# EricBAndrews/Fast-Needleman-Wunsch

Measured on AMD Instinct MI355X. Metric: GCUPS (DP cell updates/s) on NxN NW fill, bit-exact score, higher is better.
Workload: dtype int32; 1 GPU; nw_fill_262144x262144; n1=262144, n2=262144, table_bytes=274880004100, layout=row-major int32, pitch 262208, waves=auto, parallelism=single GPU, kernel=panels

## Files before the change

### fast-needleman-wunsch_amd/csrc/nw_capi.cpp

```cpp
#include <cstring>

#include "nw_host_int.h"

using namespace nwh;

extern "C" {

void nw_params_default(nw_params *p) {
    if (!p) return;
    std::memset(p, 0, sizeof(*p));
    p->match = 1;
    p->mismatch = 0;
    p->gap = -1;
    p->mode = NW_MODE_NW;
    p->waves = 0;
    p->device = -1;
}

const char *nw_strerror(int status) {
    switch (status) {
        case NW_OK: return "ok";
        case NW_ERR_ARG: return "invalid argument";
        case NW_ERR_HIP: return "HIP runtime error";
        case NW_ERR_OOM: return "out of device memory";
        case NW_ERR_TIMEOUT: return "in-kernel hand-off watchdog expired";
        case NW_ERR_NODEVICE: return "no gfx950 device";
        case NW_ERR_UNSUPPORTED: return "unsupported";
        case NW_ERR_TABLE: return "traceback met a cell no move reproduces (not a table of these parameters)";
        default: return "unknown status";
    }
}

const char *nw_version(void) {
    static char buf[256];
    std::snprintf(buf, sizeof buf, "libnwhip gfx950 %s", nw::kernel_variant());
    return buf;
}

int64_t nw_table_pitch(int64_t n1) { return round_up(n1 + 4, nw::kWave); }

int64_t nw_table_bytes(int64_t n1, int64_t n2) {
    return round_up(n2 + 1, nw::kWave) * nw_table_pitch(n1) * (int64_t)sizeof(int32_t);
}

int64_t nw_table_offset(void) { return nw::kWave - 1; }

int64_t nw_strip_lds_bytes(int32_t substrips, int32_t strip_waves) {
    if (!nw::shape_ok(substrips, strip_waves)) return -1;
    return nw::lds_bytes(substrips, strip_waves);
}

int64_t nw_panel_lds_bytes(int32_t substrips, int32_t strip_waves) {
    if (!nw::panel_shape_ok(substrips, strip_waves)) return -1;
    return nw::panel_lds_bytes(substrips, strip_waves);
}

int64_t nw_ctx_workspace_bytes(int64_t n1, int64_t n2, int32_t waves) {
    Shape s = make_shape(n1, n2, waves, 0, 0, 256, 1);
    return s.M * s.gstride * 8 + nw::rowpack_len((int32_t)s.nblocks) * 16 +
           s.waves * nw::kScratchWords * 4 + 16;
}

int nw_ctx_create(int device, nw_ctx **out) {
    if (!out) return NW_ERR_ARG;
    *out = nullptr;
    int ndev = 0;
    if (hipGetDeviceCount(&ndev) != hipSuccess || ndev == 0) return NW_ERR_NODEVICE;
    if (device < 0) NW_HIP_TRY(hipGetDevice(&device));
    if (device >= ndev) return NW_ERR_ARG;
    NW_HIP_TRY(hipSetDevice(device));
    hipDeviceProp_t prop;
    NW_HIP_TRY(hipGetDeviceProperties(&prop, device));
    if (std::strncmp(prop.gcnArchName, "gfx950", 6) != 0) {
        std::fprintf(stderr, "libnwhip: device %d is %s, kernels are built for gfx950\n", device,
                     prop.gcnArchName);
        return NW_ERR_NODEVICE;
    }
    nw_ctx *c = new nw_ctx();
    c->device = device;
    c->cus = prop.multiProcessorCount;
    if (hipMalloc(&c->ctrl, nw::kCtrlWords * 4) != hipSuccess || hipMemset(c->ctrl, 0, nw::kCtrlWords * 4) != hipSuccess ||
        hipMalloc(&c->meta, nw::kMetaBytes) != hipSuccess || hipMemset(c->meta, 0, nw::kMetaBytes) != hipSuccess ||
        hipEventCreate(&c->ev0) != hipSuccess || hipEventCreate(&c->ev1) != hipSuccess) {
        nw_ctx_destroy(c);
        return NW_ERR_HIP;
    }
    *out = c;
    return NW_OK;
}

void nw_ctx_destroy(nw_ctx *c) {
    if (!c) return;
    (void)hipSetDevice(c->device);
    if (c->gran) (void)hipFree(c->gran);
    if (c->rowpack) (void)hipFree(c->rowpack);
    if (c->meta) (void)hipFree(c->meta);
    if (c->scratch) (void)hipFree(c->scratch);
    if (c->ctrl) (void)hipFree(c->ctrl);
    if (c->smax) (void)hipFree(c->smax);
    if (c->ops) (void)hipFree(c->ops);
    if (c->swinfo) (void)hipFree(c->swinfo);
    if (c->tbscratch) (void)hipFree(c->tbscratch);
    if (c->look) (void)hipFree(c->look);
    if (c->ev0) (void)hipEventDestroy(c->ev0);
    if (c->ev1) (void)hipEventDestroy(c->ev1);
    delete c;
}

int nw_ctx_status(nw_ctx *c, void *stream) {
    if (!c) return NW_ERR_ARG;
    NW_HIP_TRY(hipSetDevice(c->device));
    uint32_t w[nw::kCtrlWords] = {};
    NW_HIP_TRY(hipMemcpyAsync(w, c->ctrl, sizeof w, hipMemcpyDeviceToHost, (hipStream_t)stream));
    NW_HIP_TRY(hipStreamSynchronize((hipStream_t)stream));
    const bool failed = (w[1] != 0 && w[13] == 0) || w[8] != 0;
    if (w[8] != 0 || w[12] != 0) {
        for (int k = 0; k < 5; ++k) c->last_failure[k] = w[8 + k];
        if (w[1] != 0 && w[13] == 0) c->last_failure[4] = w[12] + 1;
    } else if (w[1] != 0 && w[13] == 0) {
        c->last_failure[0] = w[1];
        c->last_failure[1] = w[2];
        c->last_failure[2] = w[3];
        c->last_failure[3] = w[4];
        c->last_failure[4] = 1;
    }
    if (failed) {
        static const uint32_t cleared[nw::kCtrlWords - 8] = {0, 0, 0, 0, 0, 1, 0, 0};
        NW_HIP_TRY(hipMemcpyAsync(c->ctrl + 8, cleared, sizeof cleared, hipMemcpyHostToDevice, (hipStream_t)stream));
        NW_HIP_TRY(hipStreamSynchronize((hipStream_t)stream));
    }
    return failed ? NW_ERR_TIMEOUT : NW_OK;
}

int nw_debug_ctrl(nw_ctx *c, uint32_t *out8) {
    if (!c || !out8) return NW_ERR_ARG;
    NW_HIP_TRY(hipSetDevice(c->device));
    NW_HIP_TRY(hipDeviceSynchronize());
    NW_HIP_TRY(hipMemcpy(out8, c->ctrl, 32, hipMemcpyDeviceToHost));
    return NW_OK;
}

int nw_debug_failure(nw_ctx *c, uint32_t *out5) {
    if (!c || !out5) return NW_ERR_ARG;
    NW_HIP_TRY(hipSetDevice(c->device));
    NW_HIP_TRY(hipDeviceSynchronize());
    uint32_t w[nw::kCtrlWords] = {};
    NW_HIP_TRY(hipMemcpy(w, c->ctrl, sizeof w, hipMemcpyDeviceToHost));
    if (w[8] != 0 || w[12] != 0) {
        for (int k = 0; k < 5; ++k) out5[k] = w[8 + k];
        if (w[1] != 0 && w[13] == 0) out5[4] = w[12] + 1;
    } else
        for (int k = 0; k < 5; ++k) out5[k] = c->last_failure[k];
    return NW_OK;
}

int nw_debug_set_trace(nw_ctx *c, void *d_trace) {
    if (!c) return NW_ERR_ARG;
    c->trace = (uint64_t *)d_trace;
    return NW_OK;
}

int32_t nw_debug_trace_words(void) { return nw::kTraceWords; }

}
```

### fast-needleman-wunsch_amd/csrc/nw_host_int.h

```cpp
#pragma once
#include <hip/hip_runtime.h>

#include <cstdint>
#include <cstdio>
#include <cstdlib>
#include <vector>

#include "nw_hip.h"
#include "nw_internal.h"

struct nw_ctx {
    int device = 0;
    int cus = 256;
    uint64_t *gran = nullptr;
    size_t gran_cap = 0;
    void *rowpack = nullptr;
    size_t rowpack_cap = 0;
    uint8_t *meta = nullptr;
    int32_t *scratch = nullptr;
    size_t scratch_cap = 0;
    uint32_t *ctrl = nullptr;
    uint32_t tagbase = 1;
    hipEvent_t ev0 = nullptr, ev1 = nullptr;
    int last_waves = 0;
    int last_strips = 0;
    int last_sub = 0;
    int last_nc = 0;
    uint64_t *trace = nullptr;
    int32_t *smax = nullptr;
    size_t smax_cap = 0;
    uint8_t *ops = nullptr;
    size_t ops_cap = 0;
    int64_t *swinfo = nullptr;
    void *tbscratch = nullptr;
    size_t tbscratch_cap = 0;
    int last_col0 = 0;
    int last_kernel = NW_KERNEL_STRIPS;
    uint32_t last_failure[5] = {0, 0, 0, 0, 0};
    uint64_t *look = nullptr;
    size_t look_cap = 0;
    uint32_t look_tag = 1;
    int last_finish_rows = 0;
};

#define NW_HIP_TRY(expr)                                                         \
    do {                                                                         \
        hipError_t e_ = (expr);                                                  \
        if (e_ != hipSuccess) {                                                  \
            std::fprintf(stderr, "libnwhip: %s failed: %s (%s:%d)\n", #expr,     \
                         hipGetErrorString(e_), __FILE__, __LINE__);             \
            return e_ == hipErrorOutOfMemory ? NW_ERR_OOM : NW_ERR_HIP;          \
        }                                                                        \
    } while (0)

#pragma GCC visibility push(hidden)
namespace nwh {

inline int64_t round_up(int64_t x, int64_t m) { return (x + m - 1) / m * m; }

inline int grow(void **p, size_t *cap, size_t need, bool *fresh = nullptr) {
    if (fresh) *fresh = false;
    if (need <= *cap) return NW_OK;
    if (*p) (void)hipFree(*p);
    *p = nullptr;
    *cap = 0;
    need = (size_t)round_up((int64_t)need, 1 << 21);
    NW_HIP_TRY(hipMalloc(p, need));
    *cap = need;
    if (fresh) *fresh = true;
    return NW_OK;
}

inline bool env_set(const char *name) { return std::getenv(name) != nullptr; }
inline bool env_flag(const char *name) {
    const char *e = std::getenv(name);
    return e != nullptr && e[0] == '1';
}
inline int env_int(const char *name, int unset) {
    const char *e = std::getenv(name);
    return e != nullptr ? std::atoi(e) : unset;
}

inline uint64_t timeout_ticks(int32_t ms) { return (uint64_t)(ms > 0 ? ms : 20000) * 100000ull; }

struct Shape {
    int64_t nRows, nCols, nstrips, nblocks, waves, M, gstride;
    int64_t waves_max;
    int32_t K, NC;
    int32_t kernel;
};
Shape make_shape(int64_t n1, int64_t n2, int32_t waves_req, int32_t sub_req, int32_t nc_req, int cus,
                 int64_t col0, bool sw = false, int32_t kernel_req = NW_KERNEL_AUTO);
int32_t band_kernel(int32_t k);
bool shape_valid(const Shape &s);
bool valid_params(const nw_params *p);
int tb_args(int64_t n1, int64_t n2, const nw_params *p, const nw_tb_opts *o, const uint8_t *ops, int64_t ops_cap,
            const nw_alignment *out, int32_t *band, int32_t *maxwin, int32_t *aim);
bool w_range_ok(const nw_params *p, int64_t n1, int64_t i_max);
bool affine_range_ok(const nw_params *p, int32_t gap_open, int64_t n1, int64_t i_max);
bool matrix_range_ok(const nw_params *p, int32_t gap_open, int64_t max_abs, int64_t n1, int64_t i_max);
bool perm_allowed(const nw_params *p, int32_t off);
int launch_workspace(nw_ctx *c, const Shape &s, uint64_t ntags, int32_t nbl, void *stream, int64_t *qlen);
int host_device_of(int device, int *dev);
int host_ctx_acquire(int dev, nw_ctx **c);
void host_ctx_release(int dev);
int colband_layout(int64_t n1, int64_t n2, int32_t nb, int32_t r, const nw_params *p, int cus, int64_t *sf,
                   int64_t *sc, int64_t *start, int64_t *ncols);

struct DevBufs {
    std::vector<void *> v;
    ~DevBufs() {
        for (void *q : v) (void)hipFree(q);
    }
    int alloc(void **q, size_t bytes) {
        *q = nullptr;
        NW_HIP_TRY(hipMalloc(q, bytes > 0 ? bytes : 1));
        v.push_back(*q);
        return NW_OK;
    }
};
struct Events {
    hipEvent_t a = nullptr, b = nullptr;
    ~Events() {
        if (a) (void)hipEventDestroy(a);
        if (b) (void)hipEventDestroy(b);
    }
};
struct Lease {
    int dev = 0;
    bool held = false;
    nw_ctx *c = nullptr;
    int acquire(int d) {
        const int st = host_ctx_acquire(d, &c);
        dev = d;
        held = st == NW_OK;
        return st;
    }
    ~Lease() {
        if (held) host_ctx_release(dev);
    }
};
inline int have_device(const nw_params *p, int *dev) {
    int ndev = 0;
    if (hipGetDeviceCount(&ndev) != hipSuccess || ndev == 0) return NW_ERR_NODEVICE;
    return host_device_of(p->device, dev);
}

}
#pragma GCC visibility pop
```

### fast-needleman-wunsch_amd/csrc/nw_internal.h

```cpp
#pragma once
#include <stdint.h>

#include "nw_hip.h"

namespace nw {

constexpr int kWave = 64;
constexpr int kQOff = 64;
constexpr int32_t kNeg = -(1 << 29);
constexpr int kScratchWords = kWave * kWave + 2 * kWave;
constexpr int kMaxSub = 4;
constexpr int kTraceWords = 24;
constexpr uint32_t kMaxPerm = 7;
constexpr int kMetaBytes = 256 + 16 + 32;

struct FillArgs {
    int32_t *table;
    int64_t pitch;
    const void *rowpack;
    const uint8_t *s1;
    int64_t n1, n2;
    int64_t row0;
    int64_t col0;
    int32_t nstrips;
    int32_t nblocks;
    uint64_t *gran;
    int64_t gstride;
    int32_t M;
    uint32_t tagbase;
    uint32_t *ctrl;
    const uint64_t *halo_in;
    uint64_t *halo_out;
    uint32_t halo_tag;
    int32_t *scratch;
    uint64_t *trace;
    int32_t perm;
    const uint8_t *charmap;
    const uint32_t *nprof;
    int32_t match, mismatch, gap;
    int32_t flags;
    uint64_t timeout_ticks;
    int32_t sw;
    int32_t *smax;
    int32_t strip0;
    int64_t col_end;
    const uint64_t *feed_in;
    uint64_t *feed_out;
    uint32_t feed_tag;
    int32_t nbl;
    int32_t hin0, hoshift;
    int64_t tstride, qstride, hstride;
    int32_t tr;
    int32_t tr_pub;
    int32_t tr_store_pub;
    int64_t tr_y0;
    int32_t lead_sleep;
    int32_t tr_dense;
};
bool sw_shape_ok(int substrips, int strip_waves);
int launch_colband_edge(const uint64_t *feed, int32_t *table, int64_t pitch, int64_t n2, int32_t gap,
                        int64_t start, void *stream);
int launch_tband_edges(const uint64_t *feed, int32_t *table, int64_t pitch, int64_t n1, int64_t rows,
                       int32_t gap, int64_t start, void *stream);
int launch_sw_locate(const int32_t *table, int64_t pitch, int64_t n1, int64_t n2, int64_t col0,
                     int32_t strip_cols, const int32_t *smax, int32_t nstrips, uint64_t *key, int32_t *best,
                     void *stream);
int64_t sw_half_corner(int32_t match, int32_t mismatch, int64_t n1, int64_t n2, int64_t *k);
constexpr int64_t kHalfFixMax = 64;
int launch_sw_fixup(int32_t *table, int64_t pitch, int64_t n1, int64_t n2, const uint8_t *s1, const uint8_t *s2,
                    int32_t match, int32_t mismatch, int32_t gap, int64_t col0, int32_t strip_cols, int32_t *smax,
                    void *stream);
size_t sw_tb_scratch_bytes(int32_t maxwin, int32_t band);
int run_sw_traceback(const int32_t *table, int64_t pitch, int64_t n1, const uint8_t *s1, const uint8_t *s2,
                     int32_t match, int32_t mismatch, int32_t gap, int64_t end_i, int64_t end_j, uint8_t *ops,
                     int64_t ops_cap, void *scratch, int32_t maxwin, int32_t band, int64_t *info, void *stream);
int run_nw_traceback(const int32_t *table, int64_t pitch, int64_t n1, int64_t n2, const uint8_t *s1,
                     const uint8_t *s2, int32_t match, int32_t mismatch, int32_t gap, uint8_t *ops, int64_t ops_cap,
                     void *scratch, int32_t maxwin, int32_t band, int32_t aim, int64_t *info, void *stream);
int run_nw_traceback_block(const int32_t *table, int64_t pitch, int64_t n1, int64_t rows, int64_t row0,
                           const uint8_t *s1, const uint8_t *s2, int32_t match, int32_t mismatch, int32_t gap,
                           uint8_t *ops, int64_t ops_cap, void *scratch, int32_t maxwin, int32_t band, int32_t aim,
                           int64_t *info, void *stream);
int64_t tb_shift_host(int64_t k, int64_t is, int64_t js, int32_t B, int32_t aim, int64_t row0);
constexpr int32_t kTbBandDefault = 256;
constexpr int32_t kTbMaxWinDefault = 512;

int launch_charmap(const uint8_t *d_s1, int64_t n1, uint8_t *meta, void *stream);
int launch_rowpack(const uint8_t *d_s1, int64_t n1, const uint8_t *d_s2, int64_t n2, int64_t row0,
                   int32_t perm, uint8_t *meta, void *d_q, int64_t qlen, void *stream);
bool shape_ok(int substrips, int strip_waves);
int launch_fill(const FillArgs &a, int substrips, int strip_waves, int grid, void *stream);
int lds_bytes(int substrips, int strip_waves);
bool panel_shape_ok(int c, int nwaves);
int panel_lds_bytes(int c, int nwaves);
int launch_panels(const FillArgs &a, int c, int nwaves, int grid, void *stream);
int launch_link_wait(uint32_t *word, uint32_t value, uint64_t ticks, uint32_t *poison, void *stream);
int launch_ctrl_reset(uint32_t *ctrl, void *stream);
constexpr int kCtrlWords = 16;
int launch_link_signal(uint32_t *word, uint32_t value, void *stream);

struct FinishArgs {
    int32_t *table;
    int64_t pitch;
    const uint8_t *s1;
    int64_t n1;
    const uint8_t *s2;
    int64_t li0, nrows, grow0;
    int32_t match, mismatch, gap;
    uint64_t *look;
    uint32_t tag0;
    int32_t nchunks, chunk_cols;
    uint32_t *ctrl;
    uint64_t *feed_out;
    uint32_t feed_tag;
    uint64_t timeout_ticks;
};
int finish_chunk_cols(int64_t n1, int cus);
int launch_finish_rows(const FinishArgs &a, void *stream);
int64_t rowpack_len(int32_t nblocks);
const char *kernel_variant();

}
```

### fast-needleman-wunsch_amd/csrc/nw_launch.cpp

```cpp
#include <algorithm>
#include <cstring>

#include "nw_host_int.h"

using namespace nwh;

namespace {

bool fits_i8(int32_t x) { return x >= -128 && x <= 127; }

}

namespace nwh {

bool w_range_ok(const nw_params *p, int64_t n1, int64_t i_max) {
    const long long m = std::max({std::llabs(p->match), std::llabs(p->mismatch), std::llabs(p->gap)});
    return (m + std::llabs(p->gap)) * (long long)(n1 + i_max + 2) < (1LL << 28);
}

bool affine_range_ok(const nw_params *p, int32_t gap_open, int64_t n1, int64_t i_max) {
    const long long m = std::max({std::llabs(p->match), std::llabs(p->mismatch), std::llabs(p->gap)});
    return 3 * std::llabs((long long)gap_open) + (m + std::llabs(p->gap)) * (long long)(n1 + i_max + 2) < (1LL << 28);
}

bool matrix_range_ok(const nw_params *p, int32_t gap_open, int64_t max_abs, int64_t n1, int64_t i_max) {
    const long long m = std::max<long long>(max_abs, std::llabs(p->gap));
    return 3 * std::llabs((long long)gap_open) + (m + std::llabs(p->gap)) * (long long)(n1 + i_max + 2) < (1LL << 28);
}

bool perm_allowed(const nw_params *p, int32_t off) {
    return fits_i8(p->match - off) && fits_i8(p->mismatch - off) && !(p->flags & NW_FLAG_NO_PROFILE);
}

int launch_workspace(nw_ctx *c, const Shape &s, uint64_t ntags, int32_t nbl, void *stream, int64_t *qlen) {
    int st;
    const size_t gran_need = (size_t)(s.M * s.gstride) * sizeof(uint64_t);
    bool fresh = false;
    if ((st = grow((void **)&c->gran, &c->gran_cap, gran_need, &fresh)) != NW_OK) return st;
    if (fresh || (uint64_t)c->tagbase + ntags + 2u >= 0xFFFFFFF0ull) {
        NW_HIP_TRY(hipMemsetAsync(c->gran, 0, c->gran_cap, (hipStream_t)stream));
        c->tagbase = 1;
    }
    *qlen = nw::rowpack_len((int32_t)s.nblocks);
    if ((st = grow((void **)&c->rowpack, &c->rowpack_cap, (size_t)*qlen * 16 * nbl)) != NW_OK) return st;
    if ((st = grow((void **)&c->scratch, &c->scratch_cap, (size_t)s.waves * nw::kScratchWords * 4)) != NW_OK)
        return st;
    return nw::launch_ctrl_reset(c->ctrl, stream) == hipSuccess ? NW_OK : NW_ERR_HIP;
}

}

namespace {

nw::FillArgs base_args(const nw_ctx *c, const Shape &s, const nw_params *p, bool perm_ok, int64_t qlen,
                       int64_t n1) {
    nw::FillArgs a;
    std::memset(&a, 0, sizeof a);
    a.rowpack = c->rowpack;
    a.nstrips = (int32_t)s.nstrips;
    a.nblocks = (int32_t)s.nblocks;
    a.gran = c->gran;
    a.gstride = s.gstride;
    a.M = (int32_t)s.M;
    a.tagbase = c->tagbase;
    a.ctrl = c->ctrl;
    a.scratch = c->scratch;
    a.perm = perm_ok ? 1 : 0;
    a.charmap = c->meta;
    a.nprof = (const uint32_t *)(c->meta + 256);
    a.trace = c->trace;
    a.match = p->match;
    a.mismatch = p->mismatch;
    a.gap = p->gap;
    a.flags = p->flags;
    a.timeout_ticks = timeout_ticks(p->timeout_ms);
    a.nbl = 1;
    a.hin0 = 1;
    a.qstride = qlen * 16;
    a.hstride = n1 + 1;
    return a;
}

void record_launch(nw_ctx *c, const Shape &s, int64_t col0) {
    c->last_waves = (int)s.waves;
    c->last_strips = (int)s.nstrips;
    c->last_sub = s.K;
    c->last_nc = s.NC;
    c->last_col0 = (int)col0;
    c->last_kernel = s.kernel;
}

int launch_fill(nw_ctx *c, const int8_t *d_s1, int64_t n1, const int8_t *d_s2, int64_t n2, const nw_params *p,
                const nw_band *band, const nw_colband *cb, int32_t *d_t, int64_t pitch, void *stream,
                const nw_band_cycle *cy = nullptr) {
    if (!c || !d_t || n1 < 0 || n2 < 0 || n1 >= INT32_MAX || n2 >= INT32_MAX) return NW_ERR_ARG;
    nw_band cyb;
    const int32_t nbl = cy ? cy->nblk : 1;
    if (cy) {
        if (band || cb || cy->nblk < 1 || (cy->hin_first & ~1) != 0 || (cy->hout_shift & ~1) != 0 ||
            cy->row0_max < 0 || cy->row0_max >= INT32_MAX)
            return NW_ERR_ARG;
        if (!cy->halo_in && (cy->hin_first || cy->nblk > 1)) return NW_ERR_ARG;
        if (cy->nblk > 1 && (cy->t_stride < (n2 + 1) * pitch || cy->t_stride % nw::kWave != 0)) return NW_ERR_ARG;
        if ((int64_t)nbl * n2 >= INT32_MAX) return NW_ERR_ARG;
        cyb.halo_in = cy->halo_in;
        cyb.halo_out = cy->halo_out;
        cyb.tag = cy->tag;
        cyb.row0 = (uint32_t)cy->row0_max;
        band = &cyb;
    }
    if ((n1 > 0 && !d_s1) || (n2 > 0 && !d_s2)) return NW_ERR_ARG;
    if (!valid_params(p)) return NW_ERR_ARG;
    const bool sw = p->mode == NW_MODE_SW;
    if (sw && (band || cb)) return NW_ERR_UNSUPPORTED;
    if (sw && (p->flags & NW_FLAG_DEBUG_NO_CHAIN)) return NW_ERR_ARG;
    if ((p->flags & NW_FLAG_DEBUG_NO_CHAIN) && (band || cb)) return NW_ERR_ARG;
    if (band && cb) return NW_ERR_ARG;
    if (!w_range_ok(p, n1, n2 + (band ? (int64_t)band->row0 : 0))) return NW_ERR_ARG;
    int64_t col0;
    int64_t strip_first = 0, strip_count = 0, start = 0;
    if (cb) {
        if (cb->tag == 0 || (((uintptr_t)cb->feed_in | (uintptr_t)cb->feed_out) & 7u) != 0) return NW_ERR_ARG;
        int64_t ncols = 0;
        int st0 = colband_layout(n1, n2, cb->nbands, cb->r, p, c->cus, &strip_first, &strip_count, &start, &ncols);
        if (st0 != NW_OK) return st0;
        if ((cb->r > 0) != (cb->feed_in != nullptr) || (cb->r + 1 < cb->nbands) != (cb->feed_out != nullptr))
            return NW_ERR_ARG;
        if (cb->feed_out && (p->flags & 1)) return NW_ERR_ARG;
        if ((((uintptr_t)d_t + 4u) & 255u) != 0 || pitch % nw::kWave != 0 || pitch < ncols + 3) return NW_ERR_ARG;
        col0 = 1;
    } else {
        if (pitch < n1 + 1 || pitch % nw::kWave != 0) return NW_ERR_ARG;
        if ((((uintptr_t)d_t + 4u) & 255u) == 0 && n1 >= 1 && pitch >= n1 + 4)
            col0 = 1;
        else if (((uintptr_t)d_t & 255u) == 0)
            col0 = 0;
        else
            return NW_ERR_ARG;
    }
    if (band) {
        if (band->tag == 0 || (((uintptr_t)band->halo_in | (uintptr_t)band->halo_out) & 7u) != 0)
            return NW_ERR_ARG;
        if (band->halo_out && (p->flags & 1)) return NW_ERR_ARG;
    }
    NW_HIP_TRY(hipSetDevice(c->device));
    Shape s = make_shape(n1, n2, p->waves, p->substrips, p->strip_waves, c->cus, col0, sw,
                         band || cb ? band_kernel(p->kernel) : p->kernel);
    if (!shape_valid(s)) return NW_ERR_ARG;
    const bool panels = s.kernel == NW_KERNEL_PANELS;
    if (cy && panels) return NW_ERR_UNSUPPORTED;
    if (panels && (p->flags & NW_FLAG_DEBUG_NO_CHAIN)) return NW_ERR_ARG;
    if ((int64_t)s.nstrips * nbl > INT32_MAX / 2) return NW_ERR_ARG;
    if (nbl > 1) {
        s.waves = std::max<int64_t>(1, std::min<int64_t>(s.waves_max, s.nstrips * nbl));
        s.M = std::min<int64_t>(s.nstrips * nbl, s.waves + 1);
    }
    if (cb) {
        s.nstrips = strip_count;
        s.waves = std::max<int64_t>(1, std::min<int64_t>(s.waves_max, s.nstrips));
        s.M = std::min<int64_t>(s.nstrips, s.waves + 1);
    }
    if (sw && !panels && !nw::sw_shape_ok(s.K, s.NC)) return NW_ERR_UNSUPPORTED;
    const bool half = !panels && s.K == 2 && s.NC == 4;
    if (half) {
        int64_t k = 0;
        if (!sw || nw::sw_half_corner(p->match, p->mismatch, n1, n2, &k) > nw::kHalfFixMax) return NW_ERR_UNSUPPORTED;
    }
    if (s.nstrips > INT32_MAX / 2 || s.nblocks > INT32_MAX / 2) return NW_ERR_ARG;

    int st;
    int64_t qlen = 0;
    const uint64_t ntags = (uint64_t)strip_first + (uint64_t)s.nstrips * nbl;
    if ((st = launch_workspace(c, s, ntags, nbl, stream, &qlen)) != NW_OK) return st;
    const uint8_t *s1u = n1 > 0 ? (const uint8_t *)d_s1 : (const uint8_t *)c->ctrl;
    const uint8_t *s2u = n2 > 0 ? (const uint8_t *)d_s2 : (const uint8_t *)c->ctrl;
    const bool perm_ok = perm_allowed(p, sw && panels ? p->gap : 2 * p->gap);
    if (sw) {
        const size_t need = (size_t)(s.nstrips + 8) * sizeof(int32_t);
        if ((st = grow((void **)&c->smax, &c->smax_cap, need)) != NW_OK) return st;
        NW_HIP_TRY(hipMemsetAsync(c->smax, 0, need, (hipStream_t)stream));
    }
    for (int32_t b = 0; b < nbl; ++b)
        if (nw::launch_rowpack(s1u, n1, s2u + (n2 > 0 ? (int64_t)b * n2 : 0), n2, 0, perm_ok ? 1 : 0, c->meta,
                               (char *)c->rowpack + (int64_t)b * qlen * 16, qlen, stream) != hipSuccess)
            return NW_ERR_HIP;

    nw::FillArgs a = base_args(c, s, p, perm_ok, qlen, n1);
    a.table = d_t - start;
    a.pitch = pitch;
    a.col_end = start + pitch;
    a.strip0 = (int32_t)strip_first;
    a.feed_in = cb ? cb->feed_in : nullptr;
    a.feed_out = cb ? cb->feed_out : nullptr;
    a.feed_tag = cb ? cb->tag : 0u;
    a.s1 = s1u;
    a.n1 = n1;
    a.n2 = n2;
    a.col0 = col0;
    a.halo_in = band ? band->halo_in : nullptr;
    a.halo_out = band ? band->halo_out : nullptr;
    a.halo_tag = band ? band->tag : 0u;
    a.sw = sw ? 1 : 0;
    a.smax = sw ? c->smax : nullptr;
    if (cy) {
        a.nbl = nbl;
        a.hin0 = cy->hin_first;
        a.hoshift = cy->hout_shift;
        a.tstride = cy->t_stride;
    }
    if ((panels ? nw::launch_panels(a, s.K, s.NC, (int)s.waves, stream)
                : nw::launch_fill(a, s.K, s.NC, (int)s.waves, stream)) != hipSuccess)
        return NW_ERR_HIP;
    if (cb && cb->feed_in &&
        nw::launch_colband_edge(cb->feed_in, d_t, pitch, n2, p->gap, start, stream) != hipSuccess)
        return NW_ERR_HIP;
    c->tagbase += (uint32_t)ntags + 1u;
    record_launch(c, s, col0);
    if (sw) {
        if (!c->swinfo) NW_HIP_TRY(hipMalloc(&c->swinfo, 16 * sizeof(int64_t)));
        int32_t *best = c->smax + s.nstrips;
        uint64_t *key = (uint64_t *)(c->swinfo + 12);
        if (half && !(p->flags & NW_FLAG_TIMING_ONLY) && nw::launch_sw_fixup(d_t, pitch, n1, n2, (const uint8_t *)d_s1, (const uint8_t *)d_s2, p->match,
                                        p->mismatch, p->gap, col0, (int32_t)(nw::kWave * s.K * s.NC), c->smax,
                                        stream) != hipSuccess)
            return NW_ERR_HIP;
        if (nw::launch_sw_locate(d_t, pitch, n1, n2, col0, (int32_t)(nw::kWave * s.K * s.NC), c->smax,
                                 (int32_t)s.nstrips, key, best, stream) != hipSuccess)
            return NW_ERR_HIP;
    }
    return NW_OK;
}

int launch_finisher(nw_ctx *c, const int8_t *d_s1, int64_t n1, const int8_t *d_s2, const nw_params *p,
                    const nw_tband *tb, int32_t *d_t, int64_t pitch, int64_t L, int64_t Rs, uint64_t ticks,
                    void *stream) {
    nw::FinishArgs f;
    std::memset(&f, 0, sizeof f);
    f.chunk_cols = nw::finish_chunk_cols(env_flag("NW_DEBUG_FINISH_WIDE") ? INT64_MAX / 4 : n1, c->cus);
    f.nchunks = (int32_t)((n1 + f.chunk_cols - 1) / f.chunk_cols);
    const size_t need = (size_t)L * (size_t)f.nchunks * sizeof(uint64_t);
    bool fresh = false;
    int st;
    if ((st = grow((void **)&c->look, &c->look_cap, need, &fresh)) != NW_OK) return st;
    if (fresh || (uint64_t)c->look_tag + 2u * (uint64_t)L + 2u >= 0xFFFFFFF0ull) {
        NW_HIP_TRY(hipMemsetAsync(c->look, 0, c->look_cap, (hipStream_t)stream));
        c->look_tag = 1;
    }
    f.table = d_t;
    f.pitch = pitch;
    f.s1 = (const uint8_t *)d_s1;
    f.n1 = n1;
    f.s2 = (const uint8_t *)d_s2;
    f.li0 = Rs + 1;
    f.nrows = L;
    f.grow0 = tb->row0;
    f.match = p->match;
    f.mismatch = p->mismatch;
    f.gap = p->gap;
    f.look = c->look;
    f.tag0 = c->look_tag;
    f.ctrl = c->ctrl;
    f.feed_out = tb->feed_out;
    f.feed_tag = tb->tag;
    f.timeout_ticks = ticks;
    if (nw::launch_finish_rows(f, stream) != hipSuccess) return NW_ERR_HIP;
    c->look_tag += 2u * (uint32_t)L + 2u;
    return NW_OK;
}

constexpr int kTbandLeadSleep = 8;

}

extern "C" {

int nw_fill_device_async(nw_ctx *c, const int8_t *d_s1, int64_t n1, const int8_t *d_s2,
                         int64_t n2, const nw_params *p, int32_t *d_t, int64_t pitch,
                         void *stream) {
    return launch_fill(c, d_s1, n1, d_s2, n2, p, nullptr, nullptr, d_t, pitch, stream);
}

int nw_fill_band_async(nw_ctx *c, const int8_t *d_s1, int64_t n1, const int8_t *d_s2_band,
                       int64_t n2_band, const nw_params *p, const nw_band *band, int32_t *d_t,
                       int64_t pitch, void *stream) {
    if (!band) return NW_ERR_ARG;
    return launch_fill(c, d_s1, n1, d_s2_band, n2_band, p, band, nullptr, d_t, pitch, stream);
}

int nw_fill_band_cycle_async(nw_ctx *c, const int8_t *d_s1, int64_t n1, const int8_t *d_s2_blocks,
                             int64_t n2_blk, const nw_params *p, const nw_band_cycle *cy, int32_t *d_t,
                             int64_t pitch, void *stream) {
    if (!cy) return NW_ERR_ARG;
    return launch_fill(c, d_s1, n1, d_s2_blocks, n2_blk, p, nullptr, nullptr, d_t, pitch, stream, cy);
}

int nw_fill_colband_async(nw_ctx *c, const int8_t *d_s1, int64_t n1, const int8_t *d_s2, int64_t n2,
                          const nw_params *p, const nw_colband *band, int32_t *d_t, int64_t pitch,
                          void *stream) {
    if (!band) return NW_ERR_ARG;
    return launch_fill(c, d_s1, n1, d_s2, n2, p, nullptr, band, d_t, pitch, stream);
}

int nw_fill_tband_async(nw_ctx *c, const int8_t *d_s1, int64_t n1, const int8_t *d_s2, int64_t R,
                        const nw_params *p, const nw_tband *tb, int32_t *d_t, int64_t pitch, void *stream) {
    if (!c || !d_t || !tb || !d_s1 || !d_s2 || n1 < 1 || R < 1 || n1 >= INT32_MAX || R >= INT32_MAX ||
        tb->row0 < 0 || tb->row0 + R >= INT32_MAX)
        return NW_ERR_ARG;
    if (!valid_params(p)) return NW_ERR_ARG;
    if (p->mode != NW_MODE_NW || p->kernel == NW_KERNEL_PANELS) return NW_ERR_UNSUPPORTED;
    int tC = 4, tNC = 1;
    if (p->substrips != 0 || p->strip_waves != 0) {
        tC = p->substrips ? p->substrips : 4;
        tNC = p->strip_waves ? p->strip_waves : 1;
        if (!((tC == 4 && tNC == 1) || (tC == 2 && tNC == 2))) return NW_ERR_UNSUPPORTED;
    }
    if (tb->tag == 0 || (((uintptr_t)tb->feed_in | (uintptr_t)tb->feed_out) & 7u) != 0) return NW_ERR_ARG;
    if ((tb->flags & ~(uint32_t)NW_TBAND_DENSE_POLLS) != 0) return NW_ERR_ARG;
    if ((tb->row0 > 0) != (tb->feed_in != nullptr)) return NW_ERR_ARG;
    if (tb->feed_out && (p->flags & 1)) return NW_ERR_ARG;
    if ((p->flags & NW_FLAG_DEBUG_NO_CHAIN) && (tb->feed_in || tb->feed_out)) return NW_ERR_ARG;
    if ((((uintptr_t)d_t + 4u) & 255u) != 0 || pitch % nw::kWave != 0 || pitch < n1 + 4) return NW_ERR_ARG;
    if (!w_range_ok(p, n1, tb->row0 + R)) return NW_ERR_ARG;
    NW_HIP_TRY(hipSetDevice(c->device));
    Shape s = make_shape(R, n1, p->waves, tC, tNC, c->cus, 1, false, NW_KERNEL_STRIPS);
    if (!shape_valid(s) || s.nstrips > INT32_MAX / 2 || s.nblocks > INT32_MAX / 2) return NW_ERR_ARG;
    int64_t Rs = R, L = 0;
    if (s.nstrips > s.waves && (s.nstrips - 1) % s.waves == 0 && !(p->flags & NW_FLAG_NO_FINISH) &&
        !(p->flags & 1)) {
        L = R - 256 * (s.nstrips - 1);
        Rs = R - L;
        s = make_shape(Rs, n1, p->waves, tC, tNC, c->cus, 1, false, NW_KERNEL_STRIPS);
        if (!shape_valid(s)) return NW_ERR_ARG;
    }
    int st;
    int64_t qlen = 0;
    const uint64_t ntags = (uint64_t)s.nstrips;
    if ((st = launch_workspace(c, s, ntags, 1, stream, &qlen)) != NW_OK) return st;
    const bool perm_ok = perm_allowed(p, 2 * p->gap);
    if (nw::launch_rowpack((const uint8_t *)d_s2, R, (const uint8_t *)d_s1, n1, 0, perm_ok ? 1 : 0, c->meta,
                           c->rowpack, qlen, stream) != hipSuccess)
        return NW_ERR_HIP;
    nw::FillArgs a = base_args(c, s, p, perm_ok, qlen, n1);
    a.table = d_t;
    a.pitch = pitch;
    a.col_end = INT64_MAX;
    a.feed_in = tb->feed_in;
    a.feed_out = L > 0 ? nullptr : tb->feed_out;
    a.feed_tag = tb->tag;
    a.s1 = (const uint8_t *)d_s2 - tb->row0;
    a.n1 = tb->row0 + Rs;
    a.n2 = n1;
    a.col0 = tb->row0 + 1;
    a.tr = 1;
    a.tr_y0 = tb->row0;
    a.tr_pub = (int32_t)(Rs - 1 - 256 * (s.nstrips - 1));
    static const bool compute_pub = env_flag("NW_TR_PUB_COMPUTE");
    a.tr_store_pub = compute_pub && tNC == 1 ? 0 : 1;
    a.tr_dense = (tb->flags & NW_TBAND_DENSE_POLLS) != 0 ? 1 : 0;
    static const int lead_env = env_int("NW_LEAD_SLEEP", -1);
    a.lead_sleep = lead_env >= 0 ? lead_env : tNC != 1 ? 0 : a.tr_dense ? 0 : kTbandLeadSleep;
    if (nw::launch_fill(a, tC, tNC, (int)s.waves, stream) != hipSuccess) return NW_ERR_HIP;
    if (nw::launch_tband_edges(tb->feed_in, d_t, pitch, n1, R + 1, p->gap, tb->row0, stream) != hipSuccess)
        return NW_ERR_HIP;
    c->tagbase += (uint32_t)ntags + 1u;
    c->last_finish_rows = (int)L;
    if (L > 0 && (st = launch_finisher(c, d_s1, n1, d_s2, p, tb, d_t, pitch, L, Rs, a.timeout_ticks, stream)) != NW_OK)
        return st;
    record_launch(c, s, 1);
    return NW_OK;
}

int nw_fill_device(nw_ctx *c, const int8_t *d_s1, int64_t n1, const int8_t *d_s2, int64_t n2,
                   const nw_params *p, int32_t *d_t, int64_t pitch, void *stream,
                   nw_result *out) {
    if (!c) return NW_ERR_ARG;
    NW_HIP_TRY(hipSetDevice(c->device));
    if (out) NW_HIP_TRY(hipEventRecord(c->ev0, (hipStream_t)stream));
    int st = nw_fill_device_async(c, d_s1, n1, d_s2, n2, p, d_t, pitch, stream);
    if (st != NW_OK || !out) return st;
    NW_HIP_TRY(hipEventRecord(c->ev1, (hipStream_t)stream));
    st = nw_ctx_status(c, stream);
    std::memset(out, 0, sizeof *out);
    out->status = st;
    float ms = 0.f;
    NW_HIP_TRY(hipEventElapsedTime(&ms, c->ev0, c->ev1));
    out->kernel_ms = ms;
    out->cells = n1 * n2;
    out->table_bytes = (double)(n1 + 1) * (double)(n2 + 1) * 4.0;
    out->strips = c->last_strips;
    out->waves = c->last_waves;
    out->substrips = c->last_sub;
    out->strip_waves = c->last_nc;
    out->kernel = c->last_kernel;
    int32_t score = 0;
    if (p->mode == NW_MODE_SW) {
        uint64_t key = 0;
        NW_HIP_TRY(hipMemcpy(&score, c->smax + c->last_strips, 4, hipMemcpyDeviceToHost));
        NW_HIP_TRY(hipMemcpy(&key, c->swinfo + 12, 8, hipMemcpyDeviceToHost));
        out->end_i = score > 0 ? (int64_t)(key >> 32) : 0;
        out->end_j = score > 0 ? (int64_t)(key & 0xFFFFFFFFull) : 0;
    } else {
        NW_HIP_TRY(hipMemcpy(&score, d_t + n2 * pitch + n1, 4, hipMemcpyDeviceToHost));
        out->end_i = n2;
        out->end_j = n1;
    }
    out->score = score;
    return st;
}

}
```

### fast-needleman-wunsch_amd/csrc/nw_sw.hip

```cpp
#include <hip/hip_runtime.h>
#include <stdint.h>

#include <algorithm>

#include "nw_internal.h"

namespace nw {

__global__ __launch_bounds__(256) void nw_sw_best(const int32_t *__restrict__ smax, int32_t nstrips,
                                                  int32_t *__restrict__ best, uint64_t *__restrict__ key) {
    __shared__ int32_t red[256];
    int32_t m = 0;
    for (int32_t p = threadIdx.x; p < nstrips; p += 256) m = max(m, smax[p]);
    red[threadIdx.x] = m;
    __syncthreads();
    for (int s = 128; s > 0; s >>= 1) {
        if ((int)threadIdx.x < s) red[threadIdx.x] = max(red[threadIdx.x], red[threadIdx.x + s]);
        __syncthreads();
    }
    if (threadIdx.x == 0) {
        best[0] = red[0];
        *key = ~0ull;
    }
}

constexpr int kLocRows = 64;
constexpr int kLocMaxGrid = 4096;
__global__ __launch_bounds__(256) void nw_sw_locate(const int32_t *__restrict__ table, int64_t pitch,
                                                    int64_t n1, int64_t n2, int64_t col0, int32_t strip_cols,
                                                    const int32_t *__restrict__ smax, int32_t nstrips,
                                                    const int32_t *__restrict__ best,
                                                    uint64_t *__restrict__ key) {
    const int32_t b = *best;
    if (b <= 0) return;
    __shared__ unsigned long long kmin;
    if (threadIdx.x == 0) kmin = ~0ull;
    __syncthreads();
    const int64_t nblk = (n2 + kLocRows) / kLocRows;
    for (int64_t y = blockIdx.x; y < nblk; y += gridDim.x) {
        const int64_t r0 = y * kLocRows;
        const int nr = (int)min((int64_t)kLocRows, n2 + 1 - r0);
        for (int32_t p = 0; p < nstrips; ++p) {
            if (smax[p] != b) continue;
            for (int32_t x = threadIdx.x; x < strip_cols; x += 256) {
                const int64_t c = col0 + (int64_t)p * strip_cols + x;
                if (c > n1) break;
                const int32_t *col = table + r0 * pitch + c;
                int first = kLocRows;
#pragma unroll 16
                for (int rr = kLocRows - 1; rr >= 0; --rr) {
                    const int32_t v = rr < nr ? col[rr * pitch] : 0;
                    first = v == b ? rr : first;
                }
                if (first < kLocRows)
                    atomicMin(&kmin, ((unsigned long long)(r0 + first) << 32) | (unsigned long long)c);
            }
        }
    }
    __syncthreads();
    if (threadIdx.x == 0 && kmin != ~0ull) atomicMin((unsigned long long *)key, kmin);
}

int launch_sw_locate(const int32_t *table, int64_t pitch, int64_t n1, int64_t n2, int64_t col0,
                     int32_t strip_cols, const int32_t *smax, int32_t nstrips, uint64_t *key, int32_t *best,
                     void *stream) {
    hipStream_t s = (hipStream_t)stream;
    hipLaunchKernelGGL(nw_sw_best, dim3(1), dim3(256), 0, s, smax, nstrips, best, key);
    const int64_t grid = std::min<int64_t>((n2 + kLocRows) / kLocRows, kLocMaxGrid);
    hipLaunchKernelGGL(nw_sw_locate, dim3((unsigned)grid), dim3(256), 0, s, table, pitch, n1, n2, col0, strip_cols,
                       smax, nstrips, best, key);
    return (int)hipGetLastError();
}

__global__ __launch_bounds__(64) void nw_sw_fixup(int32_t *__restrict__ t, int64_t pitch,
                                                  const uint8_t *__restrict__ s1, const uint8_t *__restrict__ s2,
                                                  int32_t match, int32_t mismatch, int32_t gap, int64_t i0,
                                                  int64_t i1, int64_t j0, int64_t j1, int64_t col0, int32_t width,
                                                  int32_t *__restrict__ smax) {
    if (threadIdx.x != 0) return;
    for (int64_t i = i0; i <= i1; ++i) {
        int32_t left = t[i * pitch + j0 - 1];
        for (int64_t j = j0; j <= j1; ++j) {
            const int32_t d = t[(i - 1) * pitch + j - 1], u = t[(i - 1) * pitch + j];
            const int32_t sc = s1[j - 1] == s2[i - 1] ? match : mismatch;
            const int32_t v = max(max(0, d + sc), max(u + gap, left + gap));
            t[i * pitch + j] = v;
            left = v;
            atomicMax(smax + (j - col0) / width, v);
        }
    }
}

int64_t sw_half_corner(int32_t match, int32_t mismatch, int64_t n1, int64_t n2, int64_t *k) {
    const int64_t m = std::max(match, mismatch);
    if (m <= 0) {
        *k = INT64_MAX;
        return 0;
    }
    *k = (65536 + m - 1) / m;
    return std::max<int64_t>(0, n2 - *k + 1) * std::max<int64_t>(0, n1 - *k + 1);
}

int launch_sw_fixup(int32_t *table, int64_t pitch, int64_t n1, int64_t n2, const uint8_t *s1, const uint8_t *s2,
                    int32_t match, int32_t mismatch, int32_t gap, int64_t col0, int32_t strip_cols, int32_t *smax,
                    void *stream) {
    int64_t k = 0;
    if (sw_half_corner(match, mismatch, n1, n2, &k) == 0) return (int)hipSuccess;
    hipLaunchKernelGGL(nw_sw_fixup, dim3(1), dim3(64), 0, (hipStream_t)stream, table, pitch, s1, s2, match,
                       mismatch, gap, k, n2, k, n1, col0, strip_cols, smax);
    return (int)hipGetLastError();
}

constexpr int kTbR = 64;
constexpr int kTbBMax = 256;
constexpr int kTbWMax = 2 * kTbBMax + 1;
constexpr int kTbThreads = 512;
constexpr int kChain = 32;
enum : uint8_t { kCStop = 0, kCDiag = 1, kCUp = 2, kCLeft = 3, kCBad = 4 };
enum : uint32_t { kXCont = 0, kXStop = 1, kXOut = 2, kXBad = 3 };
__device__ __forceinline__ uint32_t xrec(uint32_t kind, uint32_t cnt, uint32_t r, uint32_t x) {
    return kind | (cnt << 2) | (r << 12) | (x << 19);
}

enum : int { kTbLocal = 0, kTbGlobal = 1, kTbBlock = 2 };

__host__ __device__ __forceinline__ int64_t tb_shift(int64_t k, int64_t is, int64_t js, int32_t B, int32_t aim,
                                                     int64_t row0 = 0) {
    if (!aim) return 0;
    const int64_t gi = is + row0;
    const int64_t num = js - gi, lim = B / 2;
    const int64_t mag = num < 0 ? -num : num;
    if (kTbR * mag > lim * gi) return (num < 0 ? -k : k) * lim;
    return k * kTbR * num / gi;
}

template <typename F>
__device__ __forceinline__ uint32_t tb_walk(const uint8_t *cd, int W, int x, F &&emit) {
    int r = kTbR - 1;
    uint32_t cnt = 0;
    for (;;) {
        const uint8_t c = cd[r * W + x];
        if (c == kCStop) return xrec(kXStop, cnt, r, x);
        if (c == kCBad) return xrec(kXBad, cnt, r, x);
        const int nx = c == kCUp ? x + 1 : c == kCLeft ? x - 1 : x;
        if (nx < 0 || nx >= W) return xrec(kXOut, cnt, r, x);
        emit(c == kCDiag ? 0u : c == kCUp ? 1u : 2u);
        ++cnt;
        if (c != kCLeft && r == 0) return xrec(kXCont, cnt, 0, nx);
        r = c == kCLeft ? r : r - 1;
        x = nx;
    }
}

template <int KIND>
__global__ __launch_bounds__(kTbThreads) void nw_tb_windows(const int32_t *__restrict__ table, int64_t pitch,
                                                            int64_t n1, const uint8_t *__restrict__ s1,
                                                            const uint8_t *__restrict__ s2, int32_t match,
                                                            int32_t mismatch, int32_t gap, int64_t is, int64_t js,
                                                            int32_t B, int32_t aim, int64_t row0,
                                                            uint8_t *__restrict__ codes,
                                                            uint32_t *__restrict__ exits) {
    __shared__ uint8_t cd[kTbR * kTbWMax];
    const int W = 2 * B + 1;
    const int k = blockIdx.x;
    const int64_t i0 = is - (int64_t)(k + 1) * kTbR + 1;
    const int64_t dj = js - is + i0 - B - tb_shift(k, is, js, B, aim, row0);
    const int ncell = kTbR * W;
    uint8_t *gcd = codes + (int64_t)k * ncell;
#pragma unroll 4
    for (int e = threadIdx.x; e < ncell; e += kTbThreads) {
        const int r = e / W, x = e - r * W;
        const int64_t i = i0 + r, j = dj + r + x;
        const bool in = i >= 1 && j >= 1 && j <= n1;
        const int64_t ic = in ? i : 1, jc = in ? j : 1;
        const int32_t *row = table + ic * pitch;
        const int32_t t = row[jc], td = row[jc - 1 - pitch], tu = row[jc - pitch], tl = row[jc - 1];
        const int32_t sc = s1[jc - 1] == s2[ic - 1] ? match : mismatch;
        const uint8_t mv = t == td + sc ? kCDiag : t == tu + gap ? kCUp : t == tl + gap ? kCLeft : kCBad;
        uint8_t c;
        if (KIND == kTbLocal) {
            c = in && t > 0 ? mv : kCStop;
        } else if (KIND == kTbBlock) {
            c = in ? mv
                   : i == 0 && j >= 0 && j <= n1 ? kCStop
                   : j == 0 && i > 0 ? kCUp
                                     : kCBad;
        } else {
            c = in ? mv
                   : i == 0 && j == 0 ? kCStop
                   : i == 0 && j > 0 && j <= n1 ? kCLeft
                   : j == 0 && i > 0 ? kCUp
                                     : kCBad;
        }
        cd[e] = c;
        gcd[e] = c;
    }
    __syncthreads();
    for (int x = threadIdx.x; x < W; x += kTbThreads) exits[(int64_t)k * W + x] = tb_walk(cd, W, x, [](uint32_t) {});
}

__global__ __launch_bounds__(1024) void nw_tb_chain(const uint32_t *__restrict__ exits, int32_t nwin, int32_t B,
                                                    int32_t aim, int64_t is, int64_t js, int64_t row0,
                                                    int64_t ops_cap, int64_t *__restrict__ wentry,
                                                    int64_t *__restrict__ ctl) {
    __shared__ uint32_t ex[kChain * kTbWMax];
    __shared__ int64_t st[3];
    const int W = 2 * B + 1;
    const int tid = threadIdx.x;
    if (tid == 0) {
        st[0] = B;
        st[1] = ctl[0];
        st[2] = 0;
    }
    for (int k0 = 0; k0 < nwin; k0 += kChain) {
        const int nk = min(kChain, nwin - k0);
        for (int e = tid; e < nk * W; e += 1024) ex[e] = exits[(int64_t)k0 * W + e];
        __syncthreads();
        if (tid == 0) {
            int x = (int)st[0];
            int64_t off = st[1];
            for (int kk = 0; kk < nk; ++kk) {
                const int k = k0 + kk;
                wentry[2 * k] = x;
                wentry[2 * k + 1] = off;
                const uint32_t rec = ex[kk * W + x];
                const uint32_t kind = rec & 3u, cnt = (rec >> 2) & 1023u, r = (rec >> 12) & 127u, xx = rec >> 19;
                off += cnt;
                const int64_t ck = tb_shift(k, is, js, B, aim, row0);
                x = (int)xx;
                if (kind == kXCont && k + 1 < nwin) {
                    x += (int)(tb_shift(k + 1, is, js, B, aim, row0) - ck);
                    if (x >= 0 && x < W) continue;
                }
                const int64_t i0 = is - (int64_t)(k + 1) * kTbR + 1, dj = js - is + i0 - B - ck;
                ctl[1] = off > ops_cap ? 4 : (int64_t)kind;
                ctl[2] = kind == kXCont ? i0 - 1 : i0 + r;
                ctl[3] = kind == kXCont ? dj - 1 + xx : dj + r + xx;
                ctl[4] = k + 1;
                ctl[0] = off;
                st[2] = 1;
                break;
            }
            st[0] = x;
            st[1] = off;
        }
        __syncthreads();
        if (st[2]) break;
    }
}

__global__ __launch_bounds__(256) void nw_tb_emit(const uint8_t *__restrict__ codes, int32_t B,
                                                  const int64_t *__restrict__ wentry, const int64_t *__restrict__ ctl,
                                                  uint8_t *__restrict__ ops) {
    __shared__ uint32_t cdw[kTbR * kTbWMax / 4 + 1];
    __shared__ uint8_t ob[2 * kTbR + kTbWMax + 8];
    __shared__ int32_t nop;
    const int k = blockIdx.x;
    if (k >= ctl[4] || ctl[1] == 4) return;
    const int W = 2 * B + 1, ncell = kTbR * W;
    const uint32_t *g = (const uint32_t *)(codes + (int64_t)k * ncell);
    for (int e = threadIdx.x; e < ncell / 4; e += 256) cdw[e] = g[e];
    __syncthreads();
    if (threadIdx.x == 0) {
        int q = 0;
        tb_walk((const uint8_t *)cdw, W, (int)wentry[2 * k], [&](uint32_t op) { ob[q++] = (uint8_t)op; });
        nop = q;
    }
    __syncthreads();
    const int64_t off = wentry[2 * k + 1];
    for (int m = threadIdx.x; m < nop; m += 256) ops[off + m] = ob[m];
}

size_t sw_tb_scratch_bytes(int32_t maxwin, int32_t band) {
    const size_t W = 2 * (size_t)band + 1;
    return 64 + (size_t)maxwin * (16 + 4 * W + kTbR * W);
}

static int32_t tb_steep_cap(int64_t is, int64_t js, int32_t B, int64_t row0) {
    const int64_t gi = is + row0;
    const int64_t num = js - gi, mag = num < 0 ? -num : num, lim = B / 2;
    const int64_t drift = (kTbR * mag - lim * gi) / gi;
    return drift <= 0 ? INT32_MAX : (int32_t)std::min<int64_t>(B / drift + 2, INT32_MAX);
}

template <int KIND>
static int run_traceback(const int32_t *table, int64_t pitch, int64_t n1, const uint8_t *s1, const uint8_t *s2,
                         int32_t match, int32_t mismatch, int32_t gap, int64_t end_i, int64_t end_j, uint8_t *ops,
                         int64_t ops_cap, void *scratch, int32_t maxwin, int32_t band, int32_t aim, int64_t *info,
                         void *stream, int64_t row0 = 0) {
    hipStream_t s = (hipStream_t)stream;
    for (int q = 0; q < 10; ++q) info[q] = 0;
    if (band < 1 || band > kTbBMax || maxwin < 1) return (int)hipErrorInvalidValue;
    const int W = 2 * band + 1;
    int64_t *ctl = (int64_t *)scratch;
    int64_t *wentry = ctl + 8;
    uint32_t *exits = (uint32_t *)(wentry + 2 * (size_t)maxwin);
    uint8_t *codes = (uint8_t *)(exits + (size_t)maxwin * W);
    hipError_t e = hipMemsetAsync(ctl, 0, 64, s);
    if (e != hipSuccess) return (int)e;
    int64_t ci = end_i, cj = end_j, h[8] = {0, 0, 0, 0, 0, 0, 0, 0};
    for (;;) {
        if (ci <= 0 || cj <= 0) {
            info[1] = ci;
            info[2] = cj;
            break;
        }
        int32_t nwin = (int32_t)std::min<int64_t>((ci + kTbR) / kTbR, maxwin);
        if (aim) nwin = std::min(nwin, tb_steep_cap(ci, cj, band, row0));
        hipLaunchKernelGGL(nw_tb_windows<KIND>, dim3((unsigned)nwin), dim3(kTbThreads), 0, s, table, pitch, n1, s1,
                           s2, match, mismatch, gap, ci, cj, band, aim, row0, codes, exits);
        hipLaunchKernelGGL(nw_tb_chain, dim3(1), dim3(1024), 0, s, exits, nwin, band, aim, ci, cj, row0, ops_cap,
                           wentry, ctl);
        hipLaunchKernelGGL(nw_tb_emit, dim3((unsigned)nwin), dim3(256), 0, s, codes, band, wentry, ctl, ops);
        if ((e = hipGetLastError()) != hipSuccess) return (int)e;
        if ((e = hipMemcpyAsync(h, ctl, sizeof h, hipMemcpyDeviceToHost, s)) != hipSuccess) return (int)e;
        if ((e = hipStreamSynchronize(s)) != hipSuccess) return (int)e;
        info[4] += 1;
        info[5] += nwin;
        info[0] = h[0];
        if (h[1] == kXStop) {
            info[1] = h[2];
            info[2] = h[3];
            break;
        }
        if (h[1] == kXBad || h[1] == 4) {
            info[3] = h[1] == 4 ? 1 : 2;
            info[1] = h[2];
            info[2] = h[3];
            break;
        }
        ci = h[2];
        cj = h[3];
    }
    if ((KIND == kTbGlobal || (KIND == kTbBlock && info[1] > 0)) && info[3] == 0 && (info[1] > 0 || info[2] > 0)) {
        const int64_t tail = info[1] > 0 ? info[1] : info[2];
        if (info[1] < 0 || info[2] < 0 || (info[1] > 0 && info[2] > 0)) {
            info[3] = 2;
        } else if (info[0] + tail > ops_cap) {
            info[3] = 1;
        } else {
            if ((e = hipMemsetAsync(ops + info[0], info[1] > 0 ? 1 : 2, (size_t)tail, s)) != hipSuccess)
                return (int)e;
            info[0] += tail;
            info[6] = tail;
            info[1] = info[2] = 0;
        }
    }
    return (int)hipSuccess;
}

int run_sw_traceback(const int32_t *table, int64_t pitch, int64_t n1, const uint8_t *s1, const uint8_t *s2,
                     int32_t match, int32_t mismatch, int32_t gap, int64_t end_i, int64_t end_j, uint8_t *ops,
                     int64_t ops_cap, void *scratch, int32_t maxwin, int32_t band, int64_t *info, void *stream) {
    return run_traceback<kTbLocal>(table, pitch, n1, s1, s2, match, mismatch, gap, end_i, end_j, ops, ops_cap, scratch,
                                   maxwin, band, 0, info, stream);
}

int run_nw_traceback(const int32_t *table, int64_t pitch, int64_t n1, int64_t n2, const uint8_t *s1,
                     const uint8_t *s2, int32_t match, int32_t mismatch, int32_t gap, uint8_t *ops, int64_t ops_cap,
                     void *scratch, int32_t maxwin, int32_t band, int32_t aim, int64_t *info, void *stream) {
    return run_traceback<kTbGlobal>(table, pitch, n1, s1, s2, match, mismatch, gap, n2, n1, ops, ops_cap, scratch,
                                    maxwin, band, aim, info, stream);
}

int run_nw_traceback_block(const int32_t *table, int64_t pitch, int64_t n1, int64_t rows, int64_t row0,
                           const uint8_t *s1, const uint8_t *s2, int32_t match, int32_t mismatch, int32_t gap,
                           uint8_t *ops, int64_t ops_cap, void *scratch, int32_t maxwin, int32_t band, int32_t aim,
                           int64_t *info, void *stream) {
    return run_traceback<kTbBlock>(table, pitch, n1, s1, s2, match, mismatch, gap, rows, n1, ops, ops_cap, scratch,
                                   maxwin, band, aim, info, stream, row0);
}

int64_t tb_shift_host(int64_t k, int64_t is, int64_t js, int32_t B, int32_t aim, int64_t row0) {
    return tb_shift(k, is, js, B, aim, row0);
}

}
```

### fast-needleman-wunsch_amd/csrc/nw_traceback.cpp

```cpp
#include <algorithm>
#include <cstring>

#include "nw_host_int.h"

using namespace nwh;

namespace {

int tb_workspace(nw_ctx *c, size_t ops, int64_t rows, int32_t band, int32_t *maxwin) {
    int st;
    if ((st = grow((void **)&c->ops, &c->ops_cap, ops)) != NW_OK) return st;
    *maxwin = (int32_t)std::min<int64_t>(*maxwin, rows / 64 + 1);
    return grow((void **)&c->tbscratch, &c->tbscratch_cap, nw::sw_tb_scratch_bytes(*maxwin, band));
}

int tb_elapsed(nw_ctx *c, hipStream_t s, float *ms) {
    NW_HIP_TRY(hipEventRecord(c->ev1, s));
    NW_HIP_TRY(hipStreamSynchronize(s));
    NW_HIP_TRY(hipEventElapsedTime(ms, c->ev0, c->ev1));
    return NW_OK;
}

void set_alignment(nw_alignment *out, int64_t end_i, int64_t end_j, const int64_t *info, float ms, int status) {
    out->end_i = end_i;
    out->end_j = end_j;
    out->n_ops = info[0];
    out->begin_i = info[1];
    out->begin_j = info[2];
    out->traceback_ms = ms;
    out->status = status;
}

}

extern "C" {

int nw_sw_traceback(nw_ctx *c, const int8_t *d_s1, int64_t n1, const int8_t *d_s2, int64_t n2,
                    const nw_params *p, const int32_t *d_t, int64_t pitch, int64_t end_i, int64_t end_j,
                    uint8_t *host_ops, int64_t ops_cap, nw_alignment *out) {
    if (!c || !d_t || !p || !out || n1 < 0 || n2 < 0 || end_i < 0 || end_j < 0 || end_i > n2 || end_j > n1)
        return NW_ERR_ARG;
    if ((end_j > 0 && !d_s1) || (end_i > 0 && !d_s2) || (ops_cap > 0 && !host_ops) || ops_cap < 0)
        return NW_ERR_ARG;
    if (!valid_params(p) || p->mode != NW_MODE_SW) return NW_ERR_ARG;
    NW_HIP_TRY(hipSetDevice(c->device));
    NW_HIP_TRY(hipDeviceSynchronize());
    const int32_t band = std::max(1, std::min(256, env_int("NW_TB_BAND", nw::kTbBandDefault)));
    int32_t maxwin = std::max(1, env_int("NW_TB_MAXWIN", nw::kTbMaxWinDefault));
    int st;
    const size_t need = (size_t)std::max<int64_t>(end_i + end_j + 1, 1);
    if ((st = tb_workspace(c, need, end_i, band, &maxwin)) != NW_OK) return st;
    NW_HIP_TRY(hipEventRecord(c->ev0, nullptr));
    int64_t info[10];
    const int he = nw::run_sw_traceback(d_t, pitch, n1, (const uint8_t *)d_s1, (const uint8_t *)d_s2, p->match,
                                        p->mismatch, p->gap, end_i, end_j, c->ops, (int64_t)need, c->tbscratch,
                                        maxwin, band, info, nullptr);
    if (he != hipSuccess) {
        std::fprintf(stderr, "libnwhip: SW traceback failed: %s\n", hipGetErrorString((hipError_t)he));
        return NW_ERR_HIP;
    }
    float ms = 0.f;
    if ((st = tb_elapsed(c, nullptr, &ms)) != NW_OK) return st;
    if (env_set("NW_TB_DEBUG"))
        std::fprintf(stderr, "nw_sw_traceback: %lld moves, %lld rounds, %lld windows (band %d)\n", (long long)info[0],
                     (long long)info[4], (long long)info[5], band);
    std::memset(out, 0, sizeof *out);
    set_alignment(out, end_i, end_j, info, ms, info[3] == 0 ? NW_OK : NW_ERR_HIP);
    NW_HIP_TRY(hipMemcpy(&out->score, d_t + end_i * pitch + end_j, 4, hipMemcpyDeviceToHost));
    if (info[3] != 0) return out->status;
    if (info[0] > ops_cap) return NW_ERR_ARG;
    if (info[0] > 0) {
        NW_HIP_TRY(hipMemcpy(host_ops, c->ops, (size_t)info[0], hipMemcpyDeviceToHost));
        std::reverse(host_ops, host_ops + info[0]);
    }
    return NW_OK;
}

int nw_traceback(nw_ctx *c, const int8_t *d_s1, int64_t n1, const int8_t *d_s2, int64_t n2, const nw_params *p,
                 const int32_t *d_t, int64_t pitch, const nw_tb_opts *o, void *stream, uint8_t *host_ops,
                 int64_t ops_cap, nw_alignment *out, nw_tb_stats *stats) {
    int32_t band = 0, maxwin = 0, aim = 0;
    int st = tb_args(n1, n2, p, o, host_ops, ops_cap, out, &band, &maxwin, &aim);
    if (st != NW_OK) return st;
    if (!c || !d_t || pitch < n1 + 1 || (n1 > 0 && !d_s1) || (n2 > 0 && !d_s2)) return NW_ERR_ARG;
    hipStream_t s = (hipStream_t)stream;
    NW_HIP_TRY(hipSetDevice(c->device));
    if ((st = tb_workspace(c, (size_t)std::max<int64_t>(n1 + n2, 1), n2, band, &maxwin)) != NW_OK) return st;
    NW_HIP_TRY(hipEventRecord(c->ev0, s));
    int64_t info[10];
    const int he = nw::run_nw_traceback(d_t, pitch, n1, n2, (const uint8_t *)d_s1, (const uint8_t *)d_s2, p->match,
                                        p->mismatch, p->gap, c->ops, n1 + n2, c->tbscratch, maxwin, band, aim, info,
                                        stream);
    if (he != hipSuccess) {
        std::fprintf(stderr, "libnwhip: traceback failed: %s\n", hipGetErrorString((hipError_t)he));
        return NW_ERR_HIP;
    }
    std::memset(out, 0, sizeof *out);
    out->end_i = n2;
    out->end_j = n1;
    if (stats) {
        stats->rounds = (int32_t)info[4];
        stats->windows = (int32_t)info[5];
        stats->band = band;
        stats->max_windows = maxwin;
        stats->tail_ops = info[6];
    }
    const bool ok = info[3] == 0;
    NW_HIP_TRY(hipMemcpyAsync(&out->score, d_t + n2 * pitch + n1, 4, hipMemcpyDeviceToHost, s));
    if (ok && info[0] > 0) NW_HIP_TRY(hipMemcpyAsync(host_ops, c->ops, (size_t)info[0], hipMemcpyDeviceToHost, s));
    float ms = 0.f;
    if ((st = tb_elapsed(c, s, &ms)) != NW_OK) return st;
    if (!ok) {
        out->traceback_ms = ms;
        out->status = NW_ERR_TABLE;
        return NW_ERR_TABLE;
    }
    set_alignment(out, n2, n1, info, ms, NW_OK);
    std::reverse(host_ops, host_ops + info[0]);
    return NW_OK;
}

int nw_traceback_block(nw_ctx *c, const int8_t *d_s1, int64_t n1, const int8_t *d_s2_block, int64_t rows,
                       int64_t row0, const nw_params *p, const int32_t *d_t, int64_t pitch, const nw_tb_opts *o,
                       void *stream, uint8_t *host_ops, int64_t ops_cap, nw_alignment *out, nw_tb_stats *stats) {
    int32_t band = 0, maxwin = 0, aim = 0;
    int st = tb_args(n1, rows, p, o, host_ops, ops_cap, out, &band, &maxwin, &aim);
    if (st != NW_OK) return st;
    if (row0 < 0 || row0 + rows >= INT32_MAX) return NW_ERR_ARG;
    if (!c || !d_t || pitch < n1 + 1 || (n1 > 0 && !d_s1) || (rows > 0 && !d_s2_block)) return NW_ERR_ARG;
    if (row0 == 0) {
        st = nw_traceback(c, d_s1, n1, d_s2_block, rows, p, d_t, pitch, o, stream, host_ops, ops_cap, out, stats);
        return st;
    }
    hipStream_t s = (hipStream_t)stream;
    NW_HIP_TRY(hipSetDevice(c->device));
    if ((st = tb_workspace(c, (size_t)std::max<int64_t>(n1 + rows, 1), rows, band, &maxwin)) != NW_OK) return st;
    NW_HIP_TRY(hipEventRecord(c->ev0, s));
    int64_t info[10];
    const int he = nw::run_nw_traceback_block(d_t, pitch, n1, rows, row0, (const uint8_t *)d_s1,
                                              (const uint8_t *)d_s2_block, p->match, p->mismatch, p->gap, c->ops,
                                              n1 + rows, c->tbscratch, maxwin, band, aim, info, stream);
    if (he != hipSuccess) {
        std::fprintf(stderr, "libnwhip: traceback failed: %s\n", hipGetErrorString((hipError_t)he));
        return NW_ERR_HIP;
    }
    std::memset(out, 0, sizeof *out);
    if (stats) {
        stats->rounds = (int32_t)info[4];
        stats->windows = (int32_t)info[5];
        stats->band = band;
        stats->max_windows = maxwin;
        stats->tail_ops = info[6];
    }
    const bool ok = info[3] == 0;
    NW_HIP_TRY(hipMemcpyAsync(&out->score, d_t + rows * pitch + n1, 4, hipMemcpyDeviceToHost, s));
    if (ok && info[0] > 0) NW_HIP_TRY(hipMemcpyAsync(host_ops, c->ops, (size_t)info[0], hipMemcpyDeviceToHost, s));
    float ms = 0.f;
    if ((st = tb_elapsed(c, s, &ms)) != NW_OK) return st;
    if (!ok) {
        out->end_i = row0 + rows;
        out->end_j = n1;
        out->traceback_ms = ms;
        out->status = NW_ERR_TABLE;
        return NW_ERR_TABLE;
    }
    set_alignment(out, row0 + rows, n1, info, ms, NW_OK);
    out->begin_i = row0 + info[1];
    std::reverse(host_ops, host_ops + info[0]);
    return NW_OK;
}

int64_t nw_debug_tb_shift(int64_t k, int64_t is, int64_t js, int32_t band, int32_t aim, int64_t row0) {
    return nw::tb_shift_host(k, is, js, band, aim, row0);
}

}
```

Measured before the change: 1531 GCUPS.

## Batch traceback rounds on device, stage windows via LDS, use pinned host readback

Traceback rounds now read their state from a device control block and are launched in batches of several window/chain/emit rounds before each host sync. The window kernel stages table rows and sequence bytes through LDS in double-buffered chunks, and the chain kernel prefetches exits. Status, score and SW best/key readbacks go through a pinned host buffer and are folded into one async copy, replacing separate synchronous memcpys. The fill kernel itself is unchanged, so the fill metric only feels the smaller post-fill readback overhead.

```diff
diff --git a/fast-needleman-wunsch_amd/csrc/nw_capi.cpp b/fast-needleman-wunsch_amd/csrc/nw_capi.cpp
--- a/fast-needleman-wunsch_amd/csrc/nw_capi.cpp
+++ b/fast-needleman-wunsch_amd/csrc/nw_capi.cpp
@@ -79,7 +79,9 @@
     nw_ctx *c = new nw_ctx();
     c->device = device;
     c->cus = prop.multiProcessorCount;
-    if (hipMalloc(&c->ctrl, nw::kCtrlWords * 4) != hipSuccess || hipMemset(c->ctrl, 0, nw::kCtrlWords * 4) != hipSuccess ||
+    if (hipMalloc(&c->ctrl, nw::kCtrlAllWords * 4) != hipSuccess ||
+        hipMemset(c->ctrl, 0, nw::kCtrlAllWords * 4) != hipSuccess ||
+        hipHostMalloc((void **)&c->pin, kPinWords * 4, hipHostMallocDefault) != hipSuccess ||
         hipMalloc(&c->meta, nw::kMetaBytes) != hipSuccess || hipMemset(c->meta, 0, nw::kMetaBytes) != hipSuccess ||
         hipEventCreate(&c->ev0) != hipSuccess || hipEventCreate(&c->ev1) != hipSuccess) {
         nw_ctx_destroy(c);
@@ -99,7 +101,7 @@
     if (c->ctrl) (void)hipFree(c->ctrl);
     if (c->smax) (void)hipFree(c->smax);
     if (c->ops) (void)hipFree(c->ops);
-    if (c->swinfo) (void)hipFree(c->swinfo);
+    if (c->pin) (void)hipHostFree(c->pin);
     if (c->tbscratch) (void)hipFree(c->tbscratch);
     if (c->look) (void)hipFree(c->look);
     if (c->ev0) (void)hipEventDestroy(c->ev0);
@@ -110,8 +112,8 @@
 int nw_ctx_status(nw_ctx *c, void *stream) {
     if (!c) return NW_ERR_ARG;
     NW_HIP_TRY(hipSetDevice(c->device));
-    uint32_t w[nw::kCtrlWords] = {};
-    NW_HIP_TRY(hipMemcpyAsync(w, c->ctrl, sizeof w, hipMemcpyDeviceToHost, (hipStream_t)stream));
+    uint32_t *w = c->pin + kPinCtrl;
+    NW_HIP_TRY(hipMemcpyAsync(w, c->ctrl, nw::kCtrlAllWords * 4, hipMemcpyDeviceToHost, (hipStream_t)stream));
     NW_HIP_TRY(hipStreamSynchronize((hipStream_t)stream));
     const bool failed = (w[1] != 0 && w[13] == 0) || w[8] != 0;
     if (w[8] != 0 || w[12] != 0) {
diff --git a/fast-needleman-wunsch_amd/csrc/nw_host_int.h b/fast-needleman-wunsch_amd/csrc/nw_host_int.h
--- a/fast-needleman-wunsch_amd/csrc/nw_host_int.h
+++ b/fast-needleman-wunsch_amd/csrc/nw_host_int.h
@@ -31,7 +31,7 @@
     size_t smax_cap = 0;
     uint8_t *ops = nullptr;
     size_t ops_cap = 0;
-    int64_t *swinfo = nullptr;
+    uint32_t *pin = nullptr;
     void *tbscratch = nullptr;
     size_t tbscratch_cap = 0;
     int last_col0 = 0;
@@ -57,6 +57,9 @@
 namespace nwh {
 
 inline int64_t round_up(int64_t x, int64_t m) { return (x + m - 1) / m * m; }
+
+constexpr int kPinCtrl = 0, kPinTb = 32, kPinScore = 48, kPinWords = 64;
+inline int64_t *pin_tb(nw_ctx *c) { return (int64_t *)(c->pin + kPinTb); }
 
 inline int grow(void **p, size_t *cap, size_t need, bool *fresh = nullptr) {
     if (fresh) *fresh = false;
diff --git a/fast-needleman-wunsch_amd/csrc/nw_internal.h b/fast-needleman-wunsch_amd/csrc/nw_internal.h
--- a/fast-needleman-wunsch_amd/csrc/nw_internal.h
+++ b/fast-needleman-wunsch_amd/csrc/nw_internal.h
@@ -73,15 +73,19 @@
 size_t sw_tb_scratch_bytes(int32_t maxwin, int32_t band);
 int run_sw_traceback(const int32_t *table, int64_t pitch, int64_t n1, const uint8_t *s1, const uint8_t *s2,
                      int32_t match, int32_t mismatch, int32_t gap, int64_t end_i, int64_t end_j, uint8_t *ops,
-                     int64_t ops_cap, void *scratch, int32_t maxwin, int32_t band, int64_t *info, void *stream);
+                     int64_t ops_cap, void *scratch, int32_t maxwin, int32_t band, int64_t *info, void *stream,
+                     int64_t *hctl);
 int run_nw_traceback(const int32_t *table, int64_t pitch, int64_t n1, int64_t n2, const uint8_t *s1,
                      const uint8_t *s2, int32_t match, int32_t mismatch, int32_t gap, uint8_t *ops, int64_t ops_cap,
-                     void *scratch, int32_t maxwin, int32_t band, int32_t aim, int64_t *info, void *stream);
+                     void *scratch, int32_t maxwin, int32_t band, int32_t aim, int64_t *info, void *stream,
+                     int64_t *hctl);
 int run_nw_traceback_block(const int32_t *table, int64_t pitch, int64_t n1, int64_t rows, int64_t row0,
                            const uint8_t *s1, const uint8_t *s2, int32_t match, int32_t mismatch, int32_t gap,
                            uint8_t *ops, int64_t ops_cap, void *scratch, int32_t maxwin, int32_t band, int32_t aim,
-                           int64_t *info, void *stream);
+                           int64_t *info, void *stream, int64_t *hctl);
 int64_t tb_shift_host(int64_t k, int64_t is, int64_t js, int32_t B, int32_t aim, int64_t row0);
+int32_t tb_steep_cap_host(int64_t is, int64_t js, int32_t B, int64_t row0);
+int32_t tb_batch_host();
 constexpr int32_t kTbBandDefault = 256;
 constexpr int32_t kTbMaxWinDefault = 512;
 
@@ -97,6 +101,7 @@
 int launch_link_wait(uint32_t *word, uint32_t value, uint64_t ticks, uint32_t *poison, void *stream);
 int launch_ctrl_reset(uint32_t *ctrl, void *stream);
 constexpr int kCtrlWords = 16;
+constexpr int kCtrlSwBest = kCtrlWords, kCtrlSwKey = kCtrlWords + 2, kCtrlAllWords = kCtrlWords + 4;
 int launch_link_signal(uint32_t *word, uint32_t value, void *stream);
 
 struct FinishArgs {
diff --git a/fast-needleman-wunsch_amd/csrc/nw_launch.cpp b/fast-needleman-wunsch_amd/csrc/nw_launch.cpp
--- a/fast-needleman-wunsch_amd/csrc/nw_launch.cpp
+++ b/fast-needleman-wunsch_amd/csrc/nw_launch.cpp
@@ -217,9 +217,8 @@
     c->tagbase += (uint32_t)ntags + 1u;
     record_launch(c, s, col0);
     if (sw) {
-        if (!c->swinfo) NW_HIP_TRY(hipMalloc(&c->swinfo, 16 * sizeof(int64_t)));
-        int32_t *best = c->smax + s.nstrips;
-        uint64_t *key = (uint64_t *)(c->swinfo + 12);
+        int32_t *best = (int32_t *)(c->ctrl + nw::kCtrlSwBest);
+        uint64_t *key = (uint64_t *)(c->ctrl + nw::kCtrlSwKey);
         if (half && !(p->flags & NW_FLAG_TIMING_ONLY) && nw::launch_sw_fixup(d_t, pitch, n1, n2, (const uint8_t *)d_s1, (const uint8_t *)d_s2, p->match,
                                         p->mismatch, p->gap, col0, (int32_t)(nw::kWave * s.K * s.NC), c->smax,
                                         stream) != hipSuccess)
@@ -379,6 +378,9 @@
     int st = nw_fill_device_async(c, d_s1, n1, d_s2, n2, p, d_t, pitch, stream);
     if (st != NW_OK || !out) return st;
     NW_HIP_TRY(hipEventRecord(c->ev1, (hipStream_t)stream));
+    int32_t *corner = (int32_t *)(c->pin + kPinScore);
+    if (p->mode != NW_MODE_SW)
+        NW_HIP_TRY(hipMemcpyAsync(corner, d_t + n2 * pitch + n1, 4, hipMemcpyDeviceToHost, (hipStream_t)stream));
     st = nw_ctx_status(c, stream);
     std::memset(out, 0, sizeof *out);
     out->status = st;
@@ -394,13 +396,13 @@
     out->kernel = c->last_kernel;
     int32_t score = 0;
     if (p->mode == NW_MODE_SW) {
-        uint64_t key = 0;
-        NW_HIP_TRY(hipMemcpy(&score, c->smax + c->last_strips, 4, hipMemcpyDeviceToHost));
-        NW_HIP_TRY(hipMemcpy(&key, c->swinfo + 12, 8, hipMemcpyDeviceToHost));
+        const uint32_t *w = c->pin + kPinCtrl;
+        score = (int32_t)w[nw::kCtrlSwBest];
+        const uint64_t key = (uint64_t)w[nw::kCtrlSwKey] | (uint64_t)w[nw::kCtrlSwKey + 1] << 32;
         out->end_i = score > 0 ? (int64_t)(key >> 32) : 0;
         out->end_j = score > 0 ? (int64_t)(key & 0xFFFFFFFFull) : 0;
     } else {
-        NW_HIP_TRY(hipMemcpy(&score, d_t + n2 * pitch + n1, 4, hipMemcpyDeviceToHost));
+        score = *corner;
         out->end_i = n2;
         out->end_j = n1;
     }
diff --git a/fast-needleman-wunsch_amd/csrc/nw_sw.hip b/fast-needleman-wunsch_amd/csrc/nw_sw.hip
--- a/fast-needleman-wunsch_amd/csrc/nw_sw.hip
+++ b/fast-needleman-wunsch_amd/csrc/nw_sw.hip
@@ -115,6 +115,11 @@
 constexpr int kTbBMax = 256;
 constexpr int kTbWMax = 2 * kTbBMax + 1;
 constexpr int kTbThreads = 512;
+constexpr int kTbChunk = 8;
+constexpr int kTbSW = kTbWMax + 3;
+static_assert(kTbWMax <= kTbThreads + 1 && kTbWMax + 2 <= kTbThreads + 4 && kTbSW >= kTbThreads + 4 &&
+                  kTbR % kTbChunk == 0 && 4 * (kTbChunk + 1) <= kTbThreads,
+              "nw_tb_windows' staging");
 constexpr int kChain = 32;
 enum : uint8_t { kCStop = 0, kCDiag = 1, kCUp = 2, kCLeft = 3, kCBad = 4 };
 enum : uint32_t { kXCont = 0, kXStop = 1, kXOut = 2, kXBad = 3 };
@@ -134,48 +139,105 @@
     return k * kTbR * num / gi;
 }
 
+__host__ __device__ __forceinline__ int32_t tb_steep_cap(int64_t is, int64_t js, int32_t B, int64_t row0) {
+    const int64_t gi = is + row0;
+    const int64_t num = js - gi, mag = num < 0 ? -num : num, lim = B / 2;
+    const int64_t drift = (kTbR * mag - lim * gi) / gi;
+    if (drift <= 0) return INT32_MAX;
+    const int64_t cap = B / drift + 2;
+    return cap < INT32_MAX ? (int32_t)cap : INT32_MAX;
+}
+
+__host__ __device__ __forceinline__ int32_t tb_nwin(int64_t is, int64_t js, int32_t B, int32_t aim, int64_t row0,
+                                                    int32_t maxwin) {
+    const int64_t rows = (is + kTbR) / kTbR;
+    int32_t nwin = rows < maxwin ? (int32_t)rows : maxwin;
+    if (aim) {
+        const int32_t cap = tb_steep_cap(is, js, B, row0);
+        nwin = cap < nwin ? cap : nwin;
+    }
+    return nwin;
+}
+
+enum : int { kCtlOps = 0, kCtlEnd = 1, kCtlI = 2, kCtlJ = 3, kCtlUsed = 4, kCtlRounds = 5, kCtlWins = 6, kCtlDone = 7 };
+constexpr int kTbBatch = 6;
+
+__global__ void nw_tb_begin(int64_t *__restrict__ ctl, int64_t is, int64_t js) {
+    if (threadIdx.x < 8) ctl[threadIdx.x] = threadIdx.x == kCtlI ? is : threadIdx.x == kCtlJ ? js : 0;
+}
+
 template <typename F>
 __device__ __forceinline__ uint32_t tb_walk(const uint8_t *cd, int W, int x, F &&emit) {
-    int r = kTbR - 1;
-    uint32_t cnt = 0;
+    int r = kTbR - 1, at = r * W + x;
+    uint32_t cnt = 0, c;
+    bool top;
     for (;;) {
-        const uint8_t c = cd[r * W + x];
-        if (c == kCStop) return xrec(kXStop, cnt, r, x);
-        if (c == kCBad) return xrec(kXBad, cnt, r, x);
-        const int nx = c == kCUp ? x + 1 : c == kCLeft ? x - 1 : x;
-        if (nx < 0 || nx >= W) return xrec(kXOut, cnt, r, x);
-        emit(c == kCDiag ? 0u : c == kCUp ? 1u : 2u);
-        ++cnt;
-        if (c != kCLeft && r == 0) return xrec(kXCont, cnt, 0, nx);
-        r = c == kCLeft ? r : r - 1;
-        x = nx;
-    }
-}
+        c = cd[at];
+        const int dx = (int)(c == kCUp) - (int)(c == kCLeft);
+        const int nx = x + dx;
+        const bool ok = c - 1u < 3u && (unsigned)nx < (unsigned)W;
+        const bool vert = c != kCLeft;
+        top = ok && vert && r == 0;
+        if (ok) emit(c - 1u);
+        cnt += ok;
+        x = ok ? nx : x;
+        if (!ok || top) break;
+        r -= vert;
+        at += dx - (vert ? W : 0);
+    }
+    const uint32_t kind = top ? kXCont : c == kCStop ? kXStop : c == kCBad ? kXBad : kXOut;
+    return xrec(kind, cnt, r, x);
+}
+static_assert(kCDiag == 1 && kCUp == 2 && kCLeft == 3 && kCStop == 0 && kCBad == 4, "tb_walk's code arithmetic");
 
 template <int KIND>
 __global__ __launch_bounds__(kTbThreads) void nw_tb_windows(const int32_t *__restrict__ table, int64_t pitch,
                                                             int64_t n1, const uint8_t *__restrict__ s1,
                                                             const uint8_t *__restrict__ s2, int32_t match,
-                                                            int32_t mismatch, int32_t gap, int64_t is, int64_t js,
-                                                            int32_t B, int32_t aim, int64_t row0,
+                                                            int32_t mismatch, int32_t gap, int32_t B, int32_t aim,
+                                                            int64_t row0, int32_t maxwin,
+                                                            const int64_t *__restrict__ ctl,
                                                             uint8_t *__restrict__ codes,
                                                             uint32_t *__restrict__ exits) {
     __shared__ uint8_t cd[kTbR * kTbWMax];
+    __shared__ int32_t sb[2][kTbChunk + 1][kTbSW];
+    __shared__ uint8_t c1[kTbWMax + kTbR], c2[kTbR];
+    if (ctl[kCtlDone]) return;
+    const int64_t is = ctl[kCtlI], js = ctl[kCtlJ];
     const int W = 2 * B + 1;
     const int k = blockIdx.x;
+    if (k >= tb_nwin(is, js, B, aim, row0, maxwin)) return;
     const int64_t i0 = is - (int64_t)(k + 1) * kTbR + 1;
     const int64_t dj = js - is + i0 - B - tb_shift(k, is, js, B, aim, row0);
     const int ncell = kTbR * W;
+    const int tid = threadIdx.x;
     uint8_t *gcd = codes + (int64_t)k * ncell;
-#pragma unroll 4
-    for (int e = threadIdx.x; e < ncell; e += kTbThreads) {
-        const int r = e / W, x = e - r * W;
+    for (int q = tid; q < W + kTbR - 1; q += kTbThreads) {
+        const int64_t j = dj + q;
+        c1[q] = j >= 1 && j <= n1 ? s1[j - 1] : 0;
+    }
+    if (tid < kTbR) c2[tid] = i0 + tid >= 1 ? s2[i0 + tid - 1] : 0;
+    const int SW = W + 2;
+    int32_t v[kTbChunk + 2];
+    auto cell = [&](int r, int xs) -> int32_t {
+        const int64_t i = i0 + r, j = dj + r + xs - 1;
+        return xs < SW && i >= 0 && j >= 0 && j <= n1 ? table[i * pitch + j] : 0;
+    };
+    auto load = [&](int c) {
+#pragma unroll
+        for (int rr = 0; rr <= kTbChunk; ++rr) v[rr] = cell(c * kTbChunk - 1 + rr, tid);
+        v[kTbChunk + 1] = (tid >> 2) <= kTbChunk ? cell(c * kTbChunk - 1 + (tid >> 2), kTbThreads + (tid & 3)) : 0;
+    };
+    auto store = [&](int b) {
+#pragma unroll
+        for (int rr = 0; rr <= kTbChunk; ++rr) sb[b][rr][tid] = v[rr];
+        if ((tid >> 2) <= kTbChunk) sb[b][tid >> 2][kTbThreads + (tid & 3)] = v[kTbChunk + 1];
+    };
+    auto code = [&](int b, int rl, int r, int x) {
         const int64_t i = i0 + r, j = dj + r + x;
         const bool in = i >= 1 && j >= 1 && j <= n1;
-        const int64_t ic = in ? i : 1, jc = in ? j : 1;
-        const int32_t *row = table + ic * pitch;
-        const int32_t t = row[jc], td = row[jc - 1 - pitch], tu = row[jc - pitch], tl = row[jc - 1];
-        const int32_t sc = s1[jc - 1] == s2[ic - 1] ? match : mismatch;
+        const int32_t t = sb[b][rl + 1][x + 1], tl = sb[b][rl + 1][x], td = sb[b][rl][x + 1], tu = sb[b][rl][x + 2];
+        const int32_t sc = c1[r + x] == c2[r] ? match : mismatch;
         const uint8_t mv = t == td + sc ? kCDiag : t == tu + gap ? kCUp : t == tl + gap ? kCLeft : kCBad;
         uint8_t c;
         if (KIND == kTbLocal) {
@@ -192,30 +254,55 @@
                    : j == 0 && i > 0 ? kCUp
                                      : kCBad;
         }
-        cd[e] = c;
-        gcd[e] = c;
+        cd[r * W + x] = c;
+        gcd[r * W + x] = c;
+    };
+    load(0);
+    store(0);
+    for (int c = 0; c < kTbR / kTbChunk; ++c) {
+        const bool more = c + 1 < kTbR / kTbChunk;
+        if (more) load(c + 1);
+        __syncthreads();
+        if (tid < W) {
+#pragma unroll
+            for (int rl = 0; rl < kTbChunk; ++rl) code(c & 1, rl, c * kTbChunk + rl, tid);
+        }
+        if (W > kTbThreads && tid >= 64 && tid < 64 + kTbChunk) code(c & 1, tid - 64, c * kTbChunk + tid - 64, kTbThreads);
+        if (more) store((c + 1) & 1);
     }
     __syncthreads();
     for (int x = threadIdx.x; x < W; x += kTbThreads) exits[(int64_t)k * W + x] = tb_walk(cd, W, x, [](uint32_t) {});
 }
 
-__global__ __launch_bounds__(1024) void nw_tb_chain(const uint32_t *__restrict__ exits, int32_t nwin, int32_t B,
-                                                    int32_t aim, int64_t is, int64_t js, int64_t row0,
-                                                    int64_t ops_cap, int64_t *__restrict__ wentry,
-                                                    int64_t *__restrict__ ctl) {
-    __shared__ uint32_t ex[kChain * kTbWMax];
+__global__ __launch_bounds__(1024) void nw_tb_chain(const uint32_t *__restrict__ exits, int32_t maxwin, int32_t B,
+                                                    int32_t aim, int64_t row0, int64_t ops_cap,
+                                                    int64_t *__restrict__ wentry, int64_t *__restrict__ ctl) {
+    __shared__ uint32_t ex[2][kChain * kTbWMax];
     __shared__ int64_t st[3];
     const int W = 2 * B + 1;
     const int tid = threadIdx.x;
+    const bool idle = ctl[kCtlDone] != 0;
+    const int64_t is = ctl[kCtlI], js = ctl[kCtlJ];
     if (tid == 0) {
         st[0] = B;
-        st[1] = ctl[0];
+        st[1] = ctl[kCtlOps];
         st[2] = 0;
     }
-    for (int k0 = 0; k0 < nwin; k0 += kChain) {
+    __syncthreads();
+    if (idle) {
+        if (tid == 0) ctl[kCtlUsed] = 0;
+        return;
+    }
+    const int32_t nwin = tb_nwin(is, js, B, aim, row0, maxwin);
+    auto stage = [&](int k0, int b, int t0, int nt) {
+        const int ne = min(kChain, nwin - k0) * W;
+        for (int e = t0; e < ne; e += nt) ex[b][e] = exits[(int64_t)k0 * W + e];
+    };
+    stage(0, 0, tid, 1024);
+    __syncthreads();
+    for (int k0 = 0, b = 0; k0 < nwin; k0 += kChain, b ^= 1) {
         const int nk = min(kChain, nwin - k0);
-        for (int e = tid; e < nk * W; e += 1024) ex[e] = exits[(int64_t)k0 * W + e];
-        __syncthreads();
+        if (tid >= 64 && k0 + kChain < nwin) stage(k0 + kChain, b ^ 1, tid - 64, 1024 - 64);
         if (tid == 0) {
             int x = (int)st[0];
             int64_t off = st[1];
@@ -223,7 +310,7 @@
                 const int k = k0 + kk;
                 wentry[2 * k] = x;
                 wentry[2 * k + 1] = off;
-                const uint32_t rec = ex[kk * W + x];
+                const uint32_t rec = ex[b][kk * W + x];
                 const uint32_t kind = rec & 3u, cnt = (rec >> 2) & 1023u, r = (rec >> 12) & 127u, xx = rec >> 19;
                 off += cnt;
                 const int64_t ck = tb_shift(k, is, js, B, aim, row0);
@@ -233,11 +320,17 @@
                     if (x >= 0 && x < W) continue;
                 }
                 const int64_t i0 = is - (int64_t)(k + 1) * kTbR + 1, dj = js - is + i0 - B - ck;
-                ctl[1] = off > ops_cap ? 4 : (int64_t)kind;
-                ctl[2] = kind == kXCont ? i0 - 1 : i0 + r;
-                ctl[3] = kind == kXCont ? dj - 1 + xx : dj + r + xx;
-                ctl[4] = k + 1;
-                ctl[0] = off;
+                const int64_t end = off > ops_cap ? 4 : (int64_t)kind;
+                const int64_t ni = kind == kXCont ? i0 - 1 : i0 + r;
+                const int64_t nj = kind == kXCont ? dj - 1 + xx : dj + r + xx;
+                ctl[kCtlEnd] = end;
+                ctl[kCtlI] = ni;
+                ctl[kCtlJ] = nj;
+                ctl[kCtlUsed] = k + 1;
+                ctl[kCtlOps] = off;
+                ctl[kCtlRounds] += 1;
+                ctl[kCtlWins] += nwin;
+                ctl[kCtlDone] = end == kXStop || end == kXBad || end == 4 || ni <= 0 || nj <= 0;
                 st[2] = 1;
                 break;
             }
@@ -256,7 +349,7 @@
     __shared__ uint8_t ob[2 * kTbR + kTbWMax + 8];
     __shared__ int32_t nop;
     const int k = blockIdx.x;
-    if (k >= ctl[4] || ctl[1] == 4) return;
+    if (k >= ctl[kCtlUsed] || ctl[kCtlEnd] == 4) return;
     const int W = 2 * B + 1, ncell = kTbR * W;
     const uint32_t *g = (const uint32_t *)(codes + (int64_t)k * ncell);
     for (int e = threadIdx.x; e < ncell / 4; e += 256) cdw[e] = g[e];
@@ -276,18 +369,11 @@
     return 64 + (size_t)maxwin * (16 + 4 * W + kTbR * W);
 }
 
-static int32_t tb_steep_cap(int64_t is, int64_t js, int32_t B, int64_t row0) {
-    const int64_t gi = is + row0;
-    const int64_t num = js - gi, mag = num < 0 ? -num : num, lim = B / 2;
-    const int64_t drift = (kTbR * mag - lim * gi) / gi;
-    return drift <= 0 ? INT32_MAX : (int32_t)std::min<int64_t>(B / drift + 2, INT32_MAX);
-}
-
 template <int KIND>
 static int run_traceback(const int32_t *table, int64_t pitch, int64_t n1, const uint8_t *s1, const uint8_t *s2,
                          int32_t match, int32_t mismatch, int32_t gap, int64_t end_i, int64_t end_j, uint8_t *ops,
                          int64_t ops_cap, void *scratch, int32_t maxwin, int32_t band, int32_t aim, int64_t *info,
-                         void *stream, int64_t row0 = 0) {
+                         void *stream, int64_t *hctl, int64_t row0 = 0) {
     hipStream_t s = (hipStream_t)stream;
     for (int q = 0; q < 10; ++q) info[q] = 0;
     if (band < 1 || band > kTbBMax || maxwin < 1) return (int)hipErrorInvalidValue;
@@ -296,41 +382,35 @@
     int64_t *wentry = ctl + 8;
     uint32_t *exits = (uint32_t *)(wentry + 2 * (size_t)maxwin);
     uint8_t *codes = (uint8_t *)(exits + (size_t)maxwin * W);
-    hipError_t e = hipMemsetAsync(ctl, 0, 64, s);
-    if (e != hipSuccess) return (int)e;
-    int64_t ci = end_i, cj = end_j, h[8] = {0, 0, 0, 0, 0, 0, 0, 0};
-    for (;;) {
-        if (ci <= 0 || cj <= 0) {
-            info[1] = ci;
-            info[2] = cj;
-            break;
-        }
-        int32_t nwin = (int32_t)std::min<int64_t>((ci + kTbR) / kTbR, maxwin);
-        if (aim) nwin = std::min(nwin, tb_steep_cap(ci, cj, band, row0));
-        hipLaunchKernelGGL(nw_tb_windows<KIND>, dim3((unsigned)nwin), dim3(kTbThreads), 0, s, table, pitch, n1, s1,
-                           s2, match, mismatch, gap, ci, cj, band, aim, row0, codes, exits);
-        hipLaunchKernelGGL(nw_tb_chain, dim3(1), dim3(1024), 0, s, exits, nwin, band, aim, ci, cj, row0, ops_cap,
-                           wentry, ctl);
-        hipLaunchKernelGGL(nw_tb_emit, dim3((unsigned)nwin), dim3(256), 0, s, codes, band, wentry, ctl, ops);
-        if ((e = hipGetLastError()) != hipSuccess) return (int)e;
-        if ((e = hipMemcpyAsync(h, ctl, sizeof h, hipMemcpyDeviceToHost, s)) != hipSuccess) return (int)e;
-        if ((e = hipStreamSynchronize(s)) != hipSuccess) return (int)e;
-        info[4] += 1;
-        info[5] += nwin;
-        info[0] = h[0];
-        if (h[1] == kXStop) {
-            info[1] = h[2];
-            info[2] = h[3];
-            break;
-        }
-        if (h[1] == kXBad || h[1] == 4) {
-            info[3] = h[1] == 4 ? 1 : 2;
-            info[1] = h[2];
-            info[2] = h[3];
-            break;
-        }
-        ci = h[2];
-        cj = h[3];
+    hipError_t e = hipSuccess;
+    int64_t hloc[8];
+    int64_t *h = hctl ? hctl : hloc;
+    info[1] = end_i;
+    info[2] = end_j;
+    if (end_i > 0 && end_j > 0) {
+        hipLaunchKernelGGL(nw_tb_begin, dim3(1), dim3(64), 0, s, ctl, end_i, end_j);
+        for (int64_t ci = end_i;;) {
+            const unsigned grid = (unsigned)std::min<int64_t>((ci + kTbR) / kTbR, maxwin);
+            for (int b = 0; b < kTbBatch; ++b) {
+                hipLaunchKernelGGL(nw_tb_windows<KIND>, dim3(grid), dim3(kTbThreads), 0, s, table, pitch, n1, s1, s2,
+                                   match, mismatch, gap, band, aim, row0, maxwin, ctl, codes, exits);
+                hipLaunchKernelGGL(nw_tb_chain, dim3(1), dim3(1024), 0, s, exits, maxwin, band, aim, row0, ops_cap,
+                                   wentry, ctl);
+                hipLaunchKernelGGL(nw_tb_emit, dim3(grid), dim3(256), 0, s, codes, band, wentry, ctl, ops);
+            }
+            if ((e = hipGetLastError()) != hipSuccess) return (int)e;
+            if ((e = hipMemcpyAsync(h, ctl, 64, hipMemcpyDeviceToHost, s)) != hipSuccess) return (int)e;
+            if ((e = hipStreamSynchronize(s)) != hipSuccess) return (int)e;
+            if (h[kCtlDone]) break;
+            if (h[kCtlI] <= 0 || h[kCtlI] > ci) return (int)hipErrorUnknown;
+            ci = h[kCtlI];
+        }
+        info[0] = h[kCtlOps];
+        info[1] = h[kCtlI];
+        info[2] = h[kCtlJ];
+        info[3] = h[kCtlEnd] == 4 ? 1 : h[kCtlEnd] == kXBad ? 2 : 0;
+        info[4] = h[kCtlRounds];
+        info[5] = h[kCtlWins];
     }
     if ((KIND == kTbGlobal || (KIND == kTbBlock && info[1] > 0)) && info[3] == 0 && (info[1] > 0 || info[2] > 0)) {
         const int64_t tail = info[1] > 0 ? info[1] : info[2];
@@ -351,28 +431,32 @@
 
 int run_sw_traceback(const int32_t *table, int64_t pitch, int64_t n1, const uint8_t *s1, const uint8_t *s2,
                      int32_t match, int32_t mismatch, int32_t gap, int64_t end_i, int64_t end_j, uint8_t *ops,
-                     int64_t ops_cap, void *scratch, int32_t maxwin, int32_t band, int64_t *info, void *stream) {
+                     int64_t ops_cap, void *scratch, int32_t maxwin, int32_t band, int64_t *info, void *stream,
+                     int64_t *hctl) {
     return run_traceback<kTbLocal>(table, pitch, n1, s1, s2, match, mismatch, gap, end_i, end_j, ops, ops_cap, scratch,
-                                   maxwin, band, 0, info, stream);
+                                   maxwin, band, 0, info, stream, hctl);
 }
 
 int run_nw_traceback(const int32_t *table, int64_t pitch, int64_t n1, int64_t n2, const uint8_t *s1,
                      const uint8_t *s2, int32_t match, int32_t mismatch, int32_t gap, uint8_t *ops, int64_t ops_cap,
-                     void *scratch, int32_t maxwin, int32_t band, int32_t aim, int64_t *info, void *stream) {
+                     void *scratch, int32_t maxwin, int32_t band, int32_t aim, int64_t *info, void *stream,
+                     int64_t *hctl) {
     return run_traceback<kTbGlobal>(table, pitch, n1, s1, s2, match, mismatch, gap, n2, n1, ops, ops_cap, scratch,
-                                    maxwin, band, aim, info, stream);
+                                    maxwin, band, aim, info, stream, hctl);
 }
 
 int run_nw_traceback_block(const int32_t *table, int64_t pitch, int64_t n1, int64_t rows, int64_t row0,
                            const uint8_t *s1, const uint8_t *s2, int32_t match, int32_t mismatch, int32_t gap,
                            uint8_t *ops, int64_t ops_cap, void *scratch, int32_t maxwin, int32_t band, int32_t aim,
-                           int64_t *info, void *stream) {
+                           int64_t *info, void *stream, int64_t *hctl) {
     return run_traceback<kTbBlock>(table, pitch, n1, s1, s2, match, mismatch, gap, rows, n1, ops, ops_cap, scratch,
-                                   maxwin, band, aim, info, stream, row0);
+                                   maxwin, band, aim, info, stream, hctl, row0);
 }
 
 int64_t tb_shift_host(int64_t k, int64_t is, int64_t js, int32_t B, int32_t aim, int64_t row0) {
     return tb_shift(k, is, js, B, aim, row0);
 }
-
-}
+int32_t tb_steep_cap_host(int64_t is, int64_t js, int32_t B, int64_t row0) { return tb_steep_cap(is, js, B, row0); }
+int32_t tb_batch_host() { return kTbBatch; }
+
+}
diff --git a/fast-needleman-wunsch_amd/csrc/nw_traceback.cpp b/fast-needleman-wunsch_amd/csrc/nw_traceback.cpp
--- a/fast-needleman-wunsch_amd/csrc/nw_traceback.cpp
+++ b/fast-needleman-wunsch_amd/csrc/nw_traceback.cpp
@@ -54,25 +54,28 @@
     int64_t info[10];
     const int he = nw::run_sw_traceback(d_t, pitch, n1, (const uint8_t *)d_s1, (const uint8_t *)d_s2, p->match,
                                         p->mismatch, p->gap, end_i, end_j, c->ops, (int64_t)need, c->tbscratch,
-                                        maxwin, band, info, nullptr);
+                                        maxwin, band, info, nullptr, pin_tb(c));
     if (he != hipSuccess) {
         std::fprintf(stderr, "libnwhip: SW traceback failed: %s\n", hipGetErrorString((hipError_t)he));
         return NW_ERR_HIP;
     }
+    NW_HIP_TRY(hipEventRecord(c->ev1, nullptr));
+    int32_t *score = (int32_t *)(c->pin + kPinScore);
+    NW_HIP_TRY(hipMemcpyAsync(score, d_t + end_i * pitch + end_j, 4, hipMemcpyDeviceToHost, nullptr));
+    const bool want_ops = info[3] == 0 && info[0] > 0 && info[0] <= ops_cap;
+    if (want_ops) NW_HIP_TRY(hipMemcpyAsync(host_ops, c->ops, (size_t)info[0], hipMemcpyDeviceToHost, nullptr));
+    NW_HIP_TRY(hipStreamSynchronize(nullptr));
     float ms = 0.f;
-    if ((st = tb_elapsed(c, nullptr, &ms)) != NW_OK) return st;
+    NW_HIP_TRY(hipEventElapsedTime(&ms, c->ev0, c->ev1));
     if (env_set("NW_TB_DEBUG"))
         std::fprintf(stderr, "nw_sw_traceback: %lld moves, %lld rounds, %lld windows (band %d)\n", (long long)info[0],
                      (long long)info[4], (long long)info[5], band);
     std::memset(out, 0, sizeof *out);
     set_alignment(out, end_i, end_j, info, ms, info[3] == 0 ? NW_OK : NW_ERR_HIP);
-    NW_HIP_TRY(hipMemcpy(&out->score, d_t + end_i * pitch + end_j, 4, hipMemcpyDeviceToHost));
+    out->score = *score;
     if (info[3] != 0) return out->status;
     if (info[0] > ops_cap) return NW_ERR_ARG;
-    if (info[0] > 0) {
-        NW_HIP_TRY(hipMemcpy(host_ops, c->ops, (size_t)info[0], hipMemcpyDeviceToHost));
-        std::reverse(host_ops, host_ops + info[0]);
-    }
+    if (want_ops) std::reverse(host_ops, host_ops + info[0]);
     return NW_OK;
 }
 
@@ -90,7 +93,7 @@
     int64_t info[10];
     const int he = nw::run_nw_traceback(d_t, pitch, n1, n2, (const uint8_t *)d_s1, (const uint8_t *)d_s2, p->match,
                                         p->mismatch, p->gap, c->ops, n1 + n2, c->tbscratch, maxwin, band, aim, info,
-                                        stream);
+                                        stream, pin_tb(c));
     if (he != hipSuccess) {
         std::fprintf(stderr, "libnwhip: traceback failed: %s\n", hipGetErrorString((hipError_t)he));
         return NW_ERR_HIP;
@@ -139,7 +142,7 @@
     int64_t info[10];
     const int he = nw::run_nw_traceback_block(d_t, pitch, n1, rows, row0, (const uint8_t *)d_s1,
                                               (const uint8_t *)d_s2_block, p->match, p->mismatch, p->gap, c->ops,
-                                              n1 + rows, c->tbscratch, maxwin, band, aim, info, stream);
+                                              n1 + rows, c->tbscratch, maxwin, band, aim, info, stream, pin_tb(c));
     if (he != hipSuccess) {
         std::fprintf(stderr, "libnwhip: traceback failed: %s\n", hipGetErrorString((hipError_t)he));
         return NW_ERR_HIP;
@@ -174,4 +177,10 @@
     return nw::tb_shift_host(k, is, js, band, aim, row0);
 }
 
+int32_t nw_debug_tb_steep_cap(int64_t is, int64_t js, int32_t band, int64_t row0) {
+    return nw::tb_steep_cap_host(is, js, band, row0);
 }
+
+int32_t nw_debug_tb_batch(void) { return nw::tb_batch_host(); }
+
+}
```

Measured after the change: 1531 GCUPS (median of 3 runs). No clear change (+0.0%).
